# Sunshine-718/AlphaZero-AL

Measured on AMD Instinct MI355X. Metric: self-play positions/sec (Connect4 n_playout=200, batch=8192 games/GPU, vl_batch=4), higher is better.
Workload: dtype f32; 1 GPU; Connect4 self-play, n_playout=200, 8192 games/GPU, vl_batch=4, evaluator=cnn; c_base=1000, use_symmetry=True, lead_in_plies=12, streams_per_gpu=1, parallelism=independent game shards x1

## Files before the change

alphazero-al_amd/csrc/nn_conv.hip:

```cpp
#include <cstdio>
#include <cstdlib>

#include "az_nn.h"
#include "nn_common.h"

namespace {

constexpr int CELLS = 42, COLS = 7;
constexpr int PCOLS = 8, PCELLS = 72;
constexpr int TS = 4;
constexpr int COUT = 64;
constexpr int CELLB = 128;

__device__ __forceinline__ void glds16(const void *gsrc, uint32_t lds_off)
{
    uint32_t keep;
    asm volatile("s_mov_b32 %0, m0\n\ts_mov_b32 m0, %2\n\ts_nop 0\n\tglobal_load_lds_dwordx4 %1, off\n\ts_mov_b32 m0, %0"
                 : "=&s"(keep) : "v"(gsrc), "s"(lds_off) : "memory");
}
__device__ __forceinline__ uint32_t lds_addr(const void *p)
{
    return static_cast<uint32_t>(reinterpret_cast<uintptr_t>((__attribute__((address_space(3))) const void *)p));
}
__device__ __forceinline__ void lds_barrier()
{
    asm volatile("s_waitcnt lgkmcnt(0)" ::: "memory");
    __builtin_amdgcn_s_barrier();
    asm volatile("" ::: "memory");
}

__device__ unsigned long long g_prof[2048 * 8];

struct EmbedIn {
    const float    *features;
    const uint16_t *emb_own, *emb_opp;
    const uint16_t *pos;
    const int32_t  *gather;
    const uint64_t *bb_p1, *bb_p2;
    const int32_t  *turn, *sym;
};

template <int CIN, bool NORM, bool RESID, bool EMBED = false>
__global__ void __launch_bounds__(256, 2) k_conv_block(const uint16_t *x, const uint16_t *w, const uint16_t *bias,
                                                       const uint16_t *gamma, const uint16_t *beta, uint16_t *y,
                                                       int64_t B, float eps, int dbg, const int64_t *batch_dev, EmbedIn em)
{
    static_assert(!EMBED || (CIN == 32 && !NORM && !RESID), "the embedding is fused into the stem only");
    const int64_t rows_total = B;
    if (batch_dev != nullptr && *batch_dev < B) B = *batch_dev;
    constexpr int K = 9 * CIN;
    constexpr int KSTEPS = K / 32;
    constexpr int KPT = CIN / 32;
    constexpr int VPC = CIN / 8;
    constexpr int VPS = CELLS * VPC;
    constexpr int PER = (VPS + 63) / 64;
    constexpr int SB = VPS * 16;
    constexpr int OVPS = CELLS * COUT / 8;
    constexpr int OPER = (OVPS + 63) / 64;
    constexpr int OSB = OVPS * 16;

    extern __shared__ __align__(16) uint8_t smem[];
    uint8_t *img = smem;
    uint8_t *rawb = smem + TS * PCELLS * CELLB;
    uint8_t *outs = rawb + 2 * TS * SB;
    float *s_gam = reinterpret_cast<float *>(outs + (RESID ? 0 : TS * OSB)), *s_bet = s_gam + CIN;
    uint8_t *dump = reinterpret_cast<uint8_t *>(s_gam + 2 * CIN);

    const int tid = threadIdx.x;
    const int lane = tid & 63;
    const int wave = __builtin_amdgcn_readfirstlane(tid >> 6);
    const int mh = wave & 1, th = wave >> 1;
    const int l15 = lane & 15, l4 = lane >> 4;

    bf16x8 aw[2][KSTEPS];
    float bia[2][4];
#pragma unroll
    for (int mt = 0; mt < 2; ++mt) {
        const int o = mh * 32 + (l15 >> 2) * 8 + mt * 4 + (l15 & 3);
#pragma unroll
        for (int s = 0; s < KSTEPS; ++s)
            aw[mt][s] = *reinterpret_cast<const bf16x8 *>(w + static_cast<size_t>(o) * K + s * 32 + l4 * 8);
#pragma unroll
        for (int r = 0; r < 4; ++r)
            bia[mt][r] = __uint_as_float(static_cast<uint32_t>(bias[mh * 32 + l4 * 8 + mt * 4 + r]) << 16);
    }
    if (NORM && tid < CIN) {
        s_gam[tid] = __uint_as_float(static_cast<uint32_t>(gamma[tid]) << 16);
        s_bet[tid] = __uint_as_float(static_cast<uint32_t>(beta[tid]) << 16);
    }
    {
        V8 z; z.w[0] = z.w[1] = z.w[2] = z.w[3] = 0;
        constexpr int NV = (TS * PCELLS * CELLB + 2 * TS * SB) / 16;
        for (int i = tid; i < NV; i += 256) reinterpret_cast<V8 *>(smem)[i] = z;
    }
    __syncthreads();

    auto swz_in = [](int cell) { return VPC == 8 ? (cell & 7) : 0; };
    const uint32_t raw_lds = lds_addr(rawb);
    if (EMBED) {
        for (int i = tid; i < CELLS * CIN / 8; i += 256)
            reinterpret_cast<V8 *>(rawb)[i] = reinterpret_cast<const V8 *>(em.pos)[i];
        __syncthreads();
    }
    auto stage_tile = [&](int64_t tile, int buf, int lane) {
        const int64_t b = tile * TS + wave;
        if (EMBED || b >= B) return;
        const uint16_t *xs = x + b * (CELLS * CIN);
#pragma unroll
        for (int i = 0; i < PER; ++i) {
            const int s = lane + 64 * i;
            if (s < VPS) {
                const int cell = s / VPC;
                glds16(xs + (cell * VPC + ((s % VPC) ^ swz_in(cell))) * 8, raw_lds + (buf * TS + wave) * SB + i * 1024);
            }
        }
    };

    const int64_t ntiles = (B + TS - 1) / TS;
    float pl_own[PER], pl_opp[PER];
    auto load_planes = [&](int64_t tile, int lane) {
        const int64_t b = tile * TS + wave;
        const bool live = b < B;
        int64_t row = !live ? 0 : (em.gather != nullptr ? em.gather[b] : b);
        if (row < 0 || row >= rows_total) row = 0;
        if (em.features != nullptr) {
            const float *fs = em.features + row * (3 * CELLS);
#pragma unroll
            for (int i = 0; i < PER; ++i) {
                const int s = lane + 64 * i;
                const bool ok = live && s < VPS;
                pl_own[i] = ok ? fs[s / VPC] : 0.0f;
                pl_opp[i] = ok ? fs[CELLS + s / VPC] : 0.0f;
            }
        } else {
            const bool p1 = em.turn[row] > 0, mir = em.sym[row] != 0;
            const uint64_t own = p1 ? em.bb_p1[row] : em.bb_p2[row], opp = p1 ? em.bb_p2[row] : em.bb_p1[row];
#pragma unroll
            for (int i = 0; i < PER; ++i) {
                const int s = lane + 64 * i;
                const bool ok = live && s < VPS;
                const int cell = ok ? s / VPC : 0;
                const int r = cell / COLS, c = cell - r * COLS;
                const int bit = (mir ? COLS - 1 - c : c) * 7 + (5 - r);
                pl_own[i] = (ok && ((own >> bit) & 1ull)) ? 1.0f : 0.0f;
                pl_opp[i] = (ok && ((opp >> bit) & 1ull)) ? 1.0f : 0.0f;
            }
        }
    };
    if (EMBED && static_cast<int64_t>(blockIdx.x) < ntiles) load_planes(blockIdx.x, lane);
    if (static_cast<int64_t>(blockIdx.x) < ntiles) stage_tile(blockIdx.x, 0, lane);
    asm volatile("s_waitcnt vmcnt(0)" ::: "memory");
    lds_barrier();
    int par = 0;
    const bool prof = dbg & 16;
    unsigned long long tp[6] = {0, 0, 0, 0, 0, 0}, tl = prof ? __builtin_amdgcn_s_memtime() : 0;
    auto stamp = [&](int k) {
        if (prof) {
            const unsigned long long now = __builtin_amdgcn_s_memtime();
            tp[k] += now - tl;
            tl = now;
        }
    };
    uint32_t img_off[PER];
#pragma unroll
    for (int i = 0; i < PER; ++i) {
        const int sl = lane + 64 * i;
        const int cell = sl / VPC;
        const int r = cell / COLS, c = cell - r * COLS;
        const int p = (r + 1) * PCOLS + (c + 1);
        const int ck = (lane % VPC) ^ swz_in(lane / VPC);
        img_off[i] = static_cast<uint32_t>((wave * PCELLS + p) * CELLB + ((ck ^ (p & 7)) << 4));
    }
    for (int64_t tile = blockIdx.x; tile < ntiles; tile += gridDim.x, par ^= 1) {
        const int64_t b0 = tile * TS;
        uint8_t *rawt = rawb + par * TS * SB;
        uint8_t *outt = RESID ? rawt : outs;
        int lane_t = lane;
        asm volatile("" : "+v"(lane_t));

        {
            const int ck = (lane_t % VPC) ^ swz_in(lane_t / VPC);
            V8 raw[PER];
            if (EMBED) {
                const V8 eo = *reinterpret_cast<const V8 *>(em.emb_own + ck * 8), ep = *reinterpret_cast<const V8 *>(em.emb_opp + ck * 8);
#pragma unroll
                for (int i = 0; i < PER; ++i) {
                    const int s = lane_t + 64 * i;
                    if (s < VPS) {
                        const V8 ps = *reinterpret_cast<const V8 *>(rawb + s * 16);
                        const f32x2 own = {pl_own[i], pl_own[i]}, opp = {pl_opp[i], pl_opp[i]};
#pragma unroll
                        for (int q = 0; q < 4; ++q) {
                            const f32x2 v = unpack2(ps.w[q]) + own * unpack2(eo.w[q]) + opp * unpack2(ep.w[q]);
                            raw[i].w[q] = pack2(v.x, v.y);
                        }
                    } else {
                        raw[i].w[0] = raw[i].w[1] = raw[i].w[2] = raw[i].w[3] = 0;
                    }
                }
            } else {
#pragma unroll
                for (int i = 0; i < PER; ++i) {
                    const int s = lane_t + 64 * i;
                    if (s < VPS) raw[i] = *reinterpret_cast<const V8 *>(rawt + wave * SB + s * 16);
                    else raw[i].w[0] = raw[i].w[1] = raw[i].w[2] = raw[i].w[3] = 0;
                }
            }
            f32x2 sc[4], sh[4];
            if (NORM) {
                f32x2 sum2 = {0.0f, 0.0f}, sq2 = {0.0f, 0.0f};
#pragma unroll
                for (int i = 0; i < PER; ++i) {
#pragma unroll
                    for (int q = 0; q < 4; ++q) {
                        const f32x2 f = unpack2(raw[i].w[q]);
                        sum2 += f;
                        sq2 = __builtin_elementwise_fma(f, f, sq2);
                    }
                }
                const float sum = wave_sum(sum2.x + sum2.y), sq = wave_sum(sq2.x + sq2.y);
                const float mean = sum * (1.0f / (CELLS * CIN));
                const float var = fmaxf(sq * (1.0f / (CELLS * CIN)) - mean * mean, 0.0f);
                const float rstd = rsqrtf(var + eps);
#pragma unroll
                for (int q = 0; q < 4; ++q) {
                    const f32x2 gq = *reinterpret_cast<const f32x2 *>(&s_gam[ck * 8 + 2 * q]);
                    const f32x2 bq = *reinterpret_cast<const f32x2 *>(&s_bet[ck * 8 + 2 * q]);
                    sc[q] = gq * f32x2{rstd, rstd};
                    sh[q] = bq - sc[q] * f32x2{mean, mean};
                }
            }
#pragma unroll
            for (int i = 0; i < PER; ++i) {
                const int s = lane_t + 64 * i;
                if (s < VPS) {
                    V8 out = raw[i];
                    if (NORM) {
#pragma unroll
                        for (int q = 0; q < 4; ++q) {
                            const f32x2 f = __builtin_elementwise_fma(unpack2(raw[i].w[q]), sc[q], sh[q]);
                            out.w[q] = pack2(f.x, f.y);
                        }
                    }
                    *reinterpret_cast<V8 *>(img + img_off[i]) = out;
                }
            }
        }
        stamp(0);
        lds_barrier();
        stamp(1);
        if (tile + gridDim.x < ntiles) {
            stage_tile(tile + gridDim.x, par ^ 1, lane_t);
            if (EMBED) load_planes(tile + gridDim.x, lane_t);
        }

        uint32_t col[3][KPT];
        {
            const uint32_t pc = static_cast<uint32_t>(2 * th * PCELLS + l15 + 9 - PCOLS - 1);
#pragma unroll
            for (int d = 0; d < 3; ++d) {
                const uint32_t p = pc + d;
                const uint32_t o = (p * CELLB + ((l4 ^ (p & 7)) << 4)) & 0xffffu;
#pragma unroll
                for (int ks = 0; ks < KPT; ++ks) col[d][ks] = o ^ (ks << 6);
            }
        }
        auto fetch = [&](int it, int tap, bf16x8 (&xf)[KPT]) {
            const int dy = tap / 3, d = tap % 3;
            const int disp = (dy * PCOLS + (it / 3) * PCELLS + (it % 3) * 16) * CELLB;
#pragma unroll
            for (int ks = 0; ks < KPT; ++ks)
                xf[ks] = *reinterpret_cast<const bf16x8 *>(&smem[col[d][ks] + disp]);
        };
        struct Epi { V8 *slot; V8 rr, o; f32x2 t, v; };
        auto epi_begin = [&](int it, Epi &e) {
            const int smp = 2 * th + it / 3, t = (it % 3) * 16 + l15;
            const int cell = (t >> 3) * COLS + (t & 7);
            const uint32_t m = (t & 7) == 7 ? 0xffffffffu : 0u;
            const uint32_t off_real = static_cast<uint32_t>(outt - smem) + smp * OSB + cell * 128 + (((mh * 4 + l4) ^ (cell & 7)) << 4);
            const uint32_t off_dump = static_cast<uint32_t>(dump - smem) + (wave * 8 + (l15 >> 3) + 2 * l4) * 16;
            e.slot = reinterpret_cast<V8 *>(&smem[(off_real & ~m) | (off_dump & m)]);
            if (RESID) e.rr = *e.slot;
        };
        auto epi_step = [&](int step, const f32x4 (&acc)[2], Epi &e) {
            const int q = step / 9;
            const f32x2 x = {acc[q >> 1][2 * (q & 1)], acc[q >> 1][2 * (q & 1) + 1]};
            switch (step % 9) {
            case 0: e.t = x * f32x2{-1.44269504f, -1.44269504f}; break;
            case 1: e.t.x = __builtin_amdgcn_exp2f(e.t.x); break;
            case 2: e.t.y = __builtin_amdgcn_exp2f(e.t.y); break;
            case 3: e.t += f32x2{1.0f, 1.0f}; break;
            case 4: e.t.x = __builtin_amdgcn_rcpf(e.t.x); break;
            case 5: e.t.y = __builtin_amdgcn_rcpf(e.t.y); break;
            case 6: e.v = x * e.t; break;
            case 7: if (RESID) e.v += unpack2(e.rr.w[q]); break;
            default: e.o.w[q] = pack2(e.v.x, e.v.y); break;
            }
        };
        auto epi_end = [&](Epi &e) { *e.slot = e.o; };

        auto block = [&](int it, f32x4 (&acc)[2], bool with_epi, const f32x4 (&pacc)[2]) {
#pragma unroll
            for (int mt = 0; mt < 2; ++mt) acc[mt] = f32x4{bia[mt][0], bia[mt][1], bia[mt][2], bia[mt][3]};
            Epi e;
            if (with_epi) epi_begin(it - 1, e);
            bf16x8 xa[KPT], xb[KPT];
            fetch(it, 0, xa);
            __builtin_amdgcn_sched_barrier(0);
#pragma unroll
            for (int tap = 0; tap < 9; ++tap) {
                bf16x8 (&cur)[KPT] = (tap & 1) ? xb : xa;
                bf16x8 (&nxt)[KPT] = (tap & 1) ? xa : xb;
                if (tap + 1 < 9) fetch(it, tap + 1, nxt);
                __builtin_amdgcn_sched_barrier(0);
#pragma unroll
                for (int ks = 0; ks < KPT; ++ks)
#pragma unroll
                    for (int mt = 0; mt < 2; ++mt) {
                        const int s = tap * KPT + ks;
                        acc[mt] = __builtin_amdgcn_mfma_f32_16x16x32_bf16(aw[mt][s], cur[ks], acc[mt], 0, 0, 0);
                        if (with_epi) {
                            __builtin_amdgcn_sched_barrier(0);
                            constexpr int PER_SLOT = 36 / (18 * KPT);
                            const int slot = (tap * KPT + ks) * 2 + mt;
#pragma unroll
                            for (int j = 0; j < PER_SLOT; ++j) epi_step(slot * PER_SLOT + j, pacc, e);
                            __builtin_amdgcn_sched_barrier(0);
                        }
                    }
            }
            if (with_epi) epi_end(e);
        };
        if (!(dbg & 1)) {
            if ((dbg >> 5) & 3) {
                if (((dbg >> 5) & 3) == 1) __builtin_amdgcn_s_setprio(1);
                else if (((dbg >> 5) & 3) == 2) __builtin_amdgcn_s_setprio(2);
                else __builtin_amdgcn_s_setprio(3);
            }
            f32x4 acc_a[2], acc_b[2];
            block(0, acc_a, false, acc_b);
            block(1, acc_b, true, acc_a);
            block(2, acc_a, true, acc_b);
            block(3, acc_b, true, acc_a);
            block(4, acc_a, true, acc_b);
            block(5, acc_b, true, acc_a);
            {
                Epi e;
                epi_begin(5, e);
#pragma unroll
                for (int step = 0; step < 36; ++step) epi_step(step, acc_b, e);
                epi_end(e);
            }
            if ((dbg >> 5) & 3) __builtin_amdgcn_s_setprio(0);
        }
        stamp(2);
        asm volatile("s_waitcnt vmcnt(0)" ::: "memory");
        stamp(3);
        lds_barrier();
        stamp(4);

        if (b0 + wave < B && !(dbg & 2)) {
            uint16_t *ys = y + (b0 + wave) * (CELLS * COUT);
#pragma unroll
            for (int i = 0; i < OPER; ++i) {
                const int s = lane_t + 64 * i;
                if (s < OVPS) {
                    const int cell = s >> 3;
                    const V8 v = *reinterpret_cast<const V8 *>(outt + wave * OSB + s * 16);
                    *reinterpret_cast<V8 *>(ys + cell * COUT + (((s & 7) ^ (cell & 7)) << 3)) = v;
                }
            }
        }
        stamp(5);
    }
    if (prof && lane == 0 && blockIdx.x < 512)
        for (int k = 0; k < 6; ++k) g_prof[(blockIdx.x * 4 + wave) * 8 + k] = tp[k];
}

int g_dbg = 0;

template <int CIN, bool NORM, bool RESID, bool EMBED = false>
int launch(const void *x, const void *w, const void *bias, const void *gamma, const void *beta, void *y, int64_t B,
           float eps, const int64_t *batch_dev, hipStream_t s, EmbedIn em = EmbedIn{})
{
    constexpr size_t smem = static_cast<size_t>(TS) * PCELLS * CELLB + 2 * static_cast<size_t>(TS) * CELLS * CIN * 2 +
                            (RESID ? 0 : static_cast<size_t>(TS) * CELLS * COUT * 2) + 2 * CIN * sizeof(float) + 512;
    auto kern = k_conv_block<CIN, NORM, RESID, EMBED>;
    static DeviceSetup setup;
    if (setup.cus({reinterpret_cast<const void *>(kern)}, static_cast<int>(smem), [&] {
            if (getenv("AZ_NN_VERBOSE") != nullptr) {
                int per_cu = 0;
                (void)hipOccupancyMaxActiveBlocksPerMultiprocessor(&per_cu, reinterpret_cast<const void *>(kern), 256, smem);
                fprintf(stderr, "[az_nn] conv block C_in=%d: %zu B LDS, %d workgroups per CU\n", CIN, smem, per_cu);
            }
        }) == 0)
        return 2;
    static const int prio = [] { const char *e = getenv("AZ_NN_CONV_PRIO"); const int v = e ? atoi(e) : 1; return v < 0 || v > 3 ? 1 : v; }();
    const int64_t ntiles = (B + TS - 1) / TS;
    static const int64_t max_grid = getenv("AZ_NN_CONV_GRID") ? atoll(getenv("AZ_NN_CONV_GRID")) : 512;
    const unsigned grid = static_cast<unsigned>(ntiles < max_grid ? ntiles : max_grid);
    hipLaunchKernelGGL(kern, dim3(grid), dim3(256), smem, s, static_cast<const uint16_t *>(x),
                       static_cast<const uint16_t *>(w), static_cast<const uint16_t *>(bias),
                       static_cast<const uint16_t *>(gamma), static_cast<const uint16_t *>(beta),
                       static_cast<uint16_t *>(y), B, eps, g_dbg | (((g_dbg >> 5) & 3) ? 0 : (prio << 5)), batch_dev, em);
    return 0;
}

}

extern "C" {

int az_nn_debug(int flags) { g_dbg = flags; return 0; }

int az_nn_conv_profile(unsigned long long *out, int n)
{
    if (n > 2048 * 8) n = 2048 * 8;
    return hipMemcpyFromSymbol(out, HIP_SYMBOL(g_prof), sizeof(unsigned long long) * n) == hipSuccess ? 0 : 2;
}

int az_nn_conv_block(const void *x, int c_in, const void *weight_ohwi, const void *bias, const void *gamma,
                     const void *beta, int residual, void *y, int64_t batch, float eps, const int64_t *batch_dev,
                     void *stream)
{
    if (batch <= 0) return 1;
    hipStream_t s = static_cast<hipStream_t>(stream);
    const bool norm = gamma != nullptr && beta != nullptr;
    if (c_in == 64 && norm && residual) return launch<64, true, true>(x, weight_ohwi, bias, gamma, beta, y, batch, eps, batch_dev, s);
    if (c_in == 64 && norm && !residual) return launch<64, true, false>(x, weight_ohwi, bias, gamma, beta, y, batch, eps, batch_dev, s);
    if (c_in == 32 && !norm && !residual) return launch<32, false, false>(x, weight_ohwi, bias, gamma, beta, y, batch, eps, batch_dev, s);
    return 1;
}

int az_nn_stem_embed(const float *features, const void *emb_own, const void *emb_opp, const void *pos,
                     const void *weight_ohwi, const void *bias, void *y, int64_t batch, const int32_t *gather,
                     const int64_t *batch_dev, void *stream)
{
    if (batch <= 0 || features == nullptr) return 1;
    EmbedIn em{features, static_cast<const uint16_t *>(emb_own), static_cast<const uint16_t *>(emb_opp),
               static_cast<const uint16_t *>(pos), gather, nullptr, nullptr, nullptr, nullptr};
    return launch<32, false, false, true>(nullptr, weight_ohwi, bias, nullptr, nullptr, y, batch, 0.0f, batch_dev,
                                          static_cast<hipStream_t>(stream), em);
}

int az_nn_stem_embed_positions(const az_nn_positions *positions, const void *emb_own, const void *emb_opp, const void *pos,
                               const void *weight_ohwi, const void *bias, void *y, int64_t batch, const int32_t *gather,
                               const int64_t *batch_dev, void *stream)
{
    if (batch <= 0 || positions == nullptr || !positions->bb_p1 || !positions->bb_p2 || !positions->turn || !positions->sym) return 1;
    EmbedIn em{nullptr, static_cast<const uint16_t *>(emb_own), static_cast<const uint16_t *>(emb_opp),
               static_cast<const uint16_t *>(pos), gather, positions->bb_p1, positions->bb_p2, positions->turn, positions->sym};
    return launch<32, false, false, true>(nullptr, weight_ohwi, bias, nullptr, nullptr, y, batch, 0.0f, batch_dev,
                                          static_cast<hipStream_t>(stream), em);
}

}
```

alphazero-al_amd/csrc/nn_model.hip:

```cpp
#include <hip/hip_runtime.h>

#include <cstdint>
#include <cstdlib>
#include <cstring>
#include <mutex>
#include <new>
#include <vector>

#include "az_nn.h"
#include "board_sym.h"

struct az_nn_model {
    int kind = AZ_NN_KIND_CONNECT4_CNN;
    bool attn_heads_fused = true;
    az_nn_model_weights w{};
    az_nn_othello_weights ow{};
};

namespace {
constexpr int64_t kTokenBytes = 42 * 64 * 2;
constexpr uint64_t kOtTok = 64 * 32 * 2, kOtMap10 = 100 * 256 * 2, kOtMap8 = 64 * 256 * 2, kOtNeck = 64 * 8 * 2;

constexpr int kKinds = 4;
struct Profile {
    std::mutex mu;
    bool on = false;
    int stride = 1;
    int64_t seen = 0;
    std::vector<hipEvent_t> start[kKinds], stop[kKinds];
    size_t used[kKinds] = {0, 0, 0, 0};
} g_prof;
constexpr size_t kProfileMax = 4096;

__device__ __forceinline__ uint64_t position_hash(uint64_t bb0, uint64_t bb1, bool p1_to_move)
{
    uint64_t x = bb0 * 0x9E3779B97F4A7C15ull;
    x ^= (bb1 + 0x7F4A7C159E3779B9ull) * 0xBF58476D1CE4E5B9ull;
    x += p1_to_move ? 0x94D049BB133111EBull : 0x2545F4914F6CDD1Dull;
    x ^= x >> 30; x *= 0xBF58476D1CE4E5B9ull;
    x ^= x >> 27; x *= 0x94D049BB133111EBull;
    x ^= x >> 31;
    return x;
}

template <bool OTHELLO>
__global__ void __launch_bounds__(256) k_hash_eval(const float *features, const uint8_t *mask, float *probs, float *wdl,
                                                   float *ml, int64_t batch, const int32_t *rows, const int64_t *n_rows)
{
    constexpr int CELLS = OTHELLO ? 64 : 42, A = OTHELLO ? 65 : 7;
    const int lane = threadIdx.x & 63;
    const int64_t b = static_cast<int64_t>(blockIdx.x) * (blockDim.x >> 6) + (threadIdx.x >> 6);
    int64_t n = batch;
    if (n_rows != nullptr && *n_rows < n) n = *n_rows;
    if (b >= n) return;
    int64_t row = rows != nullptr ? rows[b] : b;
    if (row < 0 || row >= batch) return;
    const float *f = features + row * 3 * CELLS;
    const bool in = lane < CELLS;
    const float own = in ? f[lane] : 0.0f, opp = in ? f[CELLS + lane] : 0.0f;
    const bool p1 = f[2 * CELLS] > 0.0f;
    const int bit = OTHELLO ? lane : ((lane % 7) * 7 + (5 - lane / 7));
    const bool is_p1 = in && ((p1 && own != 0.0f) || (!p1 && opp != 0.0f));
    const bool is_p2 = in && ((p1 && opp != 0.0f) || (!p1 && own != 0.0f));
    uint64_t bb0 = 0, bb1 = 0;
    if (OTHELLO) {
        bb0 = __ballot(is_p1); bb1 = __ballot(is_p2);
    } else {
        const uint64_t m1 = __ballot(is_p1), m2 = __ballot(is_p2);
        for (int c = 0; c < 42; ++c) {
            const int bt = (c % 7) * 7 + (5 - c / 7);
            bb0 |= ((m1 >> c) & 1ull) << bt;
            bb1 |= ((m2 >> c) & 1ull) << bt;
        }
        (void)bit;
    }
    const uint64_t h = position_hash(bb0, bb1, p1);
    const uint8_t *mk = mask != nullptr ? mask + row * A : nullptr;
    if (!OTHELLO) {
        if (lane < 7) {
            const float p = static_cast<float>(1 + ((h >> (4 * lane)) & 15)) / 16.0f;
            probs[row * 7 + lane] = (mk == nullptr || mk[lane]) ? p : 0.0f;
        }
    } else {
        for (int a = lane; a < 65; a += 64) {
            const int k = a >> 4, j = a & 15;
            uint64_t hk = h + 0x9E3779B97F4A7C15ull * static_cast<uint64_t>(k + 1);
            hk ^= hk >> 29; hk *= 0xBF58476D1CE4E5B9ull; hk ^= hk >> 32;
            const float p = static_cast<float>(1 + ((hk >> (4 * j)) & 15)) / 16.0f;
            probs[row * 65 + a] = (mk == nullptr || mk[a]) ? p : 0.0f;
        }
    }
    if (lane < 3) {
        const uint64_t w0 = 1 + ((h >> 28) & 31), w1 = 1 + ((h >> 33) & 31), w2 = 1 + ((h >> 38) & 31);
        const float tot = static_cast<float>(w0 + w1 + w2);
        const uint64_t mine = lane == 0 ? w0 : (lane == 1 ? w1 : w2);
        wdl[row * 3 + lane] = static_cast<float>(mine) / tot;
    }
    if (lane == 3) {
        const float v = static_cast<float>((h >> 43) & 63);
        ml[row] = OTHELLO ? (v / 32.0f - 1.0f) : (v / 2.0f);
    }
}

template <bool OTHELLO>
__global__ void __launch_bounds__(256) k_hash_eval_positions(az_nn_positions pos, const uint8_t *mask, float *probs, float *wdl,
                                                             float *ml, int64_t batch, const int32_t *rows, const int64_t *n_rows)
{
    constexpr int A = OTHELLO ? 65 : 7;
    const int64_t b = static_cast<int64_t>(blockIdx.x) * blockDim.x + threadIdx.x;
    int64_t n = batch;
    if (n_rows != nullptr && *n_rows < n) n = *n_rows;
    if (b >= n) return;
    const int64_t row = rows != nullptr ? rows[b] : b;
    if (row < 0 || row >= batch) return;
    uint64_t bb0 = pos.bb_p1[row], bb1 = pos.bb_p2[row];
    const int sym = pos.sym[row];
    if (OTHELLO) { bb0 = az::othello_sym(bb0, sym); bb1 = az::othello_sym(bb1, sym); }
    else if (sym) { bb0 = az::mirror_columns(bb0); bb1 = az::mirror_columns(bb1); }
    const uint64_t h = position_hash(bb0, bb1, pos.turn[row] > 0);
    const uint8_t *mk = mask != nullptr ? mask + row * A : nullptr;
    if (!OTHELLO) {
        for (int a = 0; a < 7; ++a) {
            const float p = static_cast<float>(1 + ((h >> (4 * a)) & 15)) / 16.0f;
            probs[row * 7 + a] = (mk == nullptr || mk[a]) ? p : 0.0f;
        }
    } else {
        for (int k = 0; k < 5; ++k) {
            uint64_t hk = h + 0x9E3779B97F4A7C15ull * static_cast<uint64_t>(k + 1);
            hk ^= hk >> 29; hk *= 0xBF58476D1CE4E5B9ull; hk ^= hk >> 32;
            for (int j = 0; j < 16 && k * 16 + j < 65; ++j) {
                const int a = k * 16 + j;
                const float p = static_cast<float>(1 + ((hk >> (4 * j)) & 15)) / 16.0f;
                probs[row * 65 + a] = (mk == nullptr || mk[a]) ? p : 0.0f;
            }
        }
    }
    const uint64_t w0 = 1 + ((h >> 28) & 31), w1 = 1 + ((h >> 33) & 31), w2 = 1 + ((h >> 38) & 31);
    const float tot = static_cast<float>(w0 + w1 + w2);
    wdl[row * 3 + 0] = static_cast<float>(w0) / tot;
    wdl[row * 3 + 1] = static_cast<float>(w1) / tot;
    wdl[row * 3 + 2] = static_cast<float>(w2) / tot;
    const float v = static_cast<float>((h >> 43) & 63);
    ml[row] = OTHELLO ? (v / 32.0f - 1.0f) : (v / 2.0f);
}
}

extern "C" {

int az_nn_model_create(const az_nn_model_weights *w, az_nn_model **out)
{
    if (w == nullptr || out == nullptr) return 1;
    if (w->n_blocks < 0 || w->n_blocks > AZ_NN_MAX_BLOCKS) return 1;
    if ((w->stem_frag == nullptr) != (w->stem_pmap == nullptr)) return 1;
    const void *need[] = {w->emb_own, w->emb_opp, w->pos, w->stem_w, w->stem_b, w->pre_w, w->qkvg_w,
                          w->qn_w, w->kn_w, w->o_w, w->heads.p_norm, w->heads.d_val_w};
    for (const void *p : need)
        if (p == nullptr) return 1;
    for (int i = 0; i < w->n_blocks; ++i)
        if (!w->block_w[i] || !w->block_b[i] || !w->block_gamma[i] || !w->block_beta[i]) return 1;
    auto *m = new (std::nothrow) az_nn_model();
    if (m == nullptr) return 1;
    m->w = *w;
    const char *fused = getenv("AZ_ATTN_HEADS_FUSED");
    m->attn_heads_fused = fused == nullptr || strcmp(fused, "0") != 0;
    *out = m;
    return 0;
}

int az_nn_model_create_hash(int game, az_nn_model **out)
{
    if (out == nullptr || (game != 0 && game != 1)) return 1;
    auto *m = new (std::nothrow) az_nn_model();
    if (m == nullptr) return 1;
    m->kind = game == 0 ? AZ_NN_KIND_HASH_CONNECT4 : AZ_NN_KIND_HASH_OTHELLO;
    *out = m;
    return 0;
}

int az_nn_model_create_othello(const az_nn_othello_weights *w, az_nn_model **out)
{
    if (w == nullptr || out == nullptr || w->embed_table == nullptr) return 1;
    if (w->n_body < 2 || w->n_body % 2 != 0 || w->n_convs != w->n_body + 2 || w->n_convs > AZ_NN_OTHELLO_MAX_CONVS) return 1;
    for (int i = 0; i < w->n_convs; ++i)
        if (!w->conv[i].w_packed || !w->conv[i].post_scale || !w->conv[i].post_shift) return 1;
    if (!w->dual_w16 || !w->dual_scale16 || !w->dual_shift16 || !w->heads.board_w || !w->heads.a_fc_wt) return 1;
    auto *m = new (std::nothrow) az_nn_model();
    if (m == nullptr) return 1;
    m->kind = AZ_NN_KIND_OTHELLO_CNN;
    m->ow = *w;
    *out = m;
    return 0;
}

void az_nn_model_destroy(az_nn_model *m) { delete m; }

int az_nn_model_kind(const az_nn_model *m) { return m ? m->kind : -1; }

uint64_t az_nn_model_scratch_bytes(const az_nn_model *m, int64_t batch)
{
    if (m != nullptr && m->kind == AZ_NN_KIND_OTHELLO_CNN)
        return batch > 0 ? static_cast<uint64_t>(batch) * (kOtTok + 3 * kOtMap10 + 2 * kOtMap8 + kOtNeck) : 0;
    if (m != nullptr && m->kind != AZ_NN_KIND_CONNECT4_CNN) return 0;
    return batch > 0 ? static_cast<uint64_t>(2 * batch * kTokenBytes) : 0;
}

static int forward_impl(const az_nn_model *m, const float *features, const az_nn_positions *positions, const uint8_t *mask,
                        float *probs, float *wdl, float *moves_left, int64_t batch, const int32_t *rows,
                        const int64_t *n_rows, void *scratch, uint64_t scratch_bytes, void *stream);

int az_nn_model_forward(const az_nn_model *m, const float *features, const uint8_t *mask, float *probs,
                        float *wdl, float *moves_left, int64_t batch, const int32_t *rows,
                        const int64_t *n_rows, void *scratch, uint64_t scratch_bytes, void *stream)
{
    if (features == nullptr) return 1;
    return forward_impl(m, features, nullptr, mask, probs, wdl, moves_left, batch, rows, n_rows, scratch, scratch_bytes, stream);
}

int az_nn_model_forward_positions(const az_nn_model *m, const az_nn_positions *positions, const uint8_t *mask, float *probs,
                                  float *wdl, float *moves_left, int64_t batch, const int32_t *rows,
                                  const int64_t *n_rows, void *scratch, uint64_t scratch_bytes, void *stream)
{
    if (positions == nullptr || !positions->bb_p1 || !positions->bb_p2 || !positions->turn || !positions->sym) return 1;
    return forward_impl(m, nullptr, positions, mask, probs, wdl, moves_left, batch, rows, n_rows, scratch, scratch_bytes, stream);
}

static int forward_impl(const az_nn_model *m, const float *features, const az_nn_positions *positions, const uint8_t *mask,
                        float *probs, float *wdl, float *moves_left, int64_t batch, const int32_t *rows,
                        const int64_t *n_rows, void *scratch, uint64_t scratch_bytes, void *stream)
{
    if (m == nullptr || probs == nullptr || wdl == nullptr || moves_left == nullptr) return 1;
    if (batch <= 0) return batch == 0 ? 0 : 1;
    if ((rows == nullptr) != (n_rows == nullptr)) return 1;
    if (m->kind == AZ_NN_KIND_OTHELLO_CNN) {
        if (positions == nullptr || mask == nullptr) return 1;
        if (scratch == nullptr || scratch_bytes < az_nn_model_scratch_bytes(m, batch)) return 1;
        const az_nn_othello_weights &o = m->ow;
        char *base = static_cast<char *>(scratch);
        char *tok = base; base += batch * kOtTok;
        char *map[3];
        for (auto &p : map) { p = base; base += batch * kOtMap10; }
        char *pa = base; base += batch * kOtMap8;
        char *pb = base; base += batch * kOtMap8;
        char *neck = base;
        auto conv = [&](int i, const void *x, const void *res, void *y) {
            const az_nn_othello_conv_layer &l = o.conv[i];
            return az_nn_othello_conv(x, l.w_packed, l.pre_scale, l.pre_shift, l.post_scale, l.post_shift, l.residual ? res : nullptr,
                                      y, batch, l.c_in, l.h_in, l.pad, 1, n_rows, stream);
        };
        int rc = az_nn_othello_embed(positions, mask, o.embed_table, tok, batch, rows, n_rows, stream);
        int cur = 0;
        if (rc == 0) rc = conv(0, tok, nullptr, map[cur]);
        for (int i = 1; rc == 0 && i + 1 < o.n_body; i += 2) {
            const int y1 = (cur + 1) % 3, y2 = (cur + 2) % 3;
            rc = conv(i, map[cur], nullptr, map[y1]);
            if (rc == 0) rc = conv(i + 1, map[y1], map[cur], map[y2]);
            cur = y2;
        }
        const int hid = (cur + 1) % 3;
        if (rc == 0) rc = conv(o.n_body - 1, map[cur], nullptr, map[hid]);
        if (rc == 0) rc = conv(o.n_body, map[hid], nullptr, pa);
        if (rc == 0) rc = conv(o.n_body + 1, pa, nullptr, pb);
        if (rc == 0) rc = az_nn_othello_conv_narrow(map[hid], o.dual_w16, o.dual_scale16, o.dual_shift16, neck, batch, n_rows, stream);
        if (rc == 0) rc = az_nn_othello_heads(pb, neck, &o.heads, probs, wdl, moves_left, batch, rows, n_rows, stream);
        return rc;
    }
    if (m->kind != AZ_NN_KIND_CONNECT4_CNN && positions != nullptr) {
        const dim3 grid(static_cast<unsigned>((batch + 255) / 256)), block(256);
        if (m->kind == AZ_NN_KIND_HASH_OTHELLO)
            hipLaunchKernelGGL(k_hash_eval_positions<true>, grid, block, 0, static_cast<hipStream_t>(stream), *positions, mask, probs,
                               wdl, moves_left, batch, rows, n_rows);
        else
            hipLaunchKernelGGL(k_hash_eval_positions<false>, grid, block, 0, static_cast<hipStream_t>(stream), *positions, mask, probs,
                               wdl, moves_left, batch, rows, n_rows);
        return 0;
    }
    if (m->kind != AZ_NN_KIND_CONNECT4_CNN) {
        const dim3 grid(static_cast<unsigned>((batch + 3) / 4)), block(256);
        if (m->kind == AZ_NN_KIND_HASH_OTHELLO)
            hipLaunchKernelGGL(k_hash_eval<true>, grid, block, 0, static_cast<hipStream_t>(stream), features, mask, probs, wdl,
                               moves_left, batch, rows, n_rows);
        else
            hipLaunchKernelGGL(k_hash_eval<false>, grid, block, 0, static_cast<hipStream_t>(stream), features, mask, probs, wdl,
                               moves_left, batch, rows, n_rows);
        return 0;
    }
    if (scratch == nullptr || scratch_bytes < az_nn_model_scratch_bytes(m, batch)) return 1;
    const az_nn_model_weights &w = m->w;
    char *a = static_cast<char *>(scratch);
    char *b = a + batch * kTokenBytes;
    hipStream_t hs = static_cast<hipStream_t>(stream);
    bool timed = false;
    int slot[kKinds] = {-1, -1, -1, -1};
    if (g_prof.on) {
        std::lock_guard<std::mutex> lk(g_prof.mu);
        hipStreamCaptureStatus cs = hipStreamCaptureStatusNone;
        const bool capturing = hipStreamIsCapturing(hs, &cs) == hipSuccess && cs != hipStreamCaptureStatusNone;
        if (g_prof.on && !capturing && (g_prof.seen++ % g_prof.stride) == 0) {
            timed = true;
            for (int kd = 0; kd < kKinds; ++kd)
                if (g_prof.used[kd] < g_prof.start[kd].size()) slot[kd] = static_cast<int>(g_prof.used[kd]++);
        }
    }
    auto begin = [&](int kd) { if (timed && slot[kd] >= 0) (void)hipEventRecord(g_prof.start[kd][slot[kd]], hs); };
    auto end = [&](int kd) { if (timed && slot[kd] >= 0) (void)hipEventRecord(g_prof.stop[kd][slot[kd]], hs); };
    begin(AZ_NN_PROFILE_STEM);
    int rc;
    if (w.stem_frag != nullptr && w.stem_pmap != nullptr)
        rc = positions != nullptr
            ? az_nn_stem_folded_positions(positions, w.stem_frag, w.stem_pmap, a, batch, rows, n_rows, stream)
            : az_nn_stem_folded(features, w.stem_frag, w.stem_pmap, a, batch, rows, n_rows, stream);
    else
        rc = positions != nullptr
            ? az_nn_stem_embed_positions(positions, w.emb_own, w.emb_opp, w.pos, w.stem_w, w.stem_b, a, batch, rows, n_rows, stream)
            : az_nn_stem_embed(features, w.emb_own, w.emb_opp, w.pos, w.stem_w, w.stem_b, a, batch, rows, n_rows, stream);
    end(AZ_NN_PROFILE_STEM);
    for (int i = 0; rc == 0 && i < w.n_blocks; ++i) {
        if (i == 0) begin(AZ_NN_PROFILE_CONV);
        rc = az_nn_conv_block(a, 64, w.block_w[i], w.block_b[i], w.block_gamma[i], w.block_beta[i], 1, b, batch,
                              w.eps, n_rows, stream);
        if (i == 0) end(AZ_NN_PROFILE_CONV);
        char *t = a; a = b; b = t;
    }
    if (rc == 0 && m->attn_heads_fused && !timed)
        return az_nn_attn_heads(a, w.pre_w, w.qkvg_w, w.qn_w, w.kn_w, w.o_w, &w.heads, mask, probs, wdl, moves_left, batch,
                                w.eps, rows, n_rows, stream);
    if (rc == 0) {
        begin(AZ_NN_PROFILE_ATTN);
        rc = az_nn_attn_block(a, w.pre_w, w.qkvg_w, w.qn_w, w.kn_w, w.o_w, b, batch, w.eps, n_rows, stream);
        end(AZ_NN_PROFILE_ATTN);
        char *t = a; a = b; b = t;
    }
    if (rc == 0) {
        begin(AZ_NN_PROFILE_HEADS);
        rc = az_nn_heads(a, &w.heads, mask, probs, wdl, moves_left, batch, w.eps, rows, n_rows, stream);
        end(AZ_NN_PROFILE_HEADS);
    }
    return rc;
}

int az_nn_model_profile(int enable)
{
    std::lock_guard<std::mutex> lk(g_prof.mu);
    if (enable) {
        for (int kd = 0; kd < kKinds; ++kd)
            while (g_prof.start[kd].size() < kProfileMax) {
                hipEvent_t a, b;
                if (hipEventCreate(&a) != hipSuccess || hipEventCreate(&b) != hipSuccess) return 2;
                g_prof.start[kd].push_back(a); g_prof.stop[kd].push_back(b);
            }
    }
    g_prof.on = enable != 0;
    g_prof.stride = enable > 1 ? enable : 1;
    g_prof.seen = 0;
    return 0;
}

int az_nn_model_profile_read_kernels(double out_ms[4], int64_t out_launches[4])
{
    if (out_ms == nullptr || out_launches == nullptr) return 1;
    if (hipDeviceSynchronize() != hipSuccess) return 2;
    std::lock_guard<std::mutex> lk(g_prof.mu);
    for (int kd = 0; kd < kKinds; ++kd) {
        double ms = 0.0;
        for (size_t i = 0; i < g_prof.used[kd]; ++i) {
            float t = 0.f;
            if (hipEventElapsedTime(&t, g_prof.start[kd][i], g_prof.stop[kd][i]) != hipSuccess) return 2;
            ms += t;
        }
        out_ms[kd] = ms;
        out_launches[kd] = static_cast<int64_t>(g_prof.used[kd]);
        g_prof.used[kd] = 0;
    }
    return 0;
}

int az_nn_model_profile_read(double *out_ms, int64_t *out_launches)
{
    if (out_ms == nullptr || out_launches == nullptr) return 1;
    double ms[4]; int64_t n[4];
    const int rc = az_nn_model_profile_read_kernels(ms, n);
    if (rc != 0) return rc;
    *out_ms = ms[AZ_NN_PROFILE_CONV];
    *out_launches = n[AZ_NN_PROFILE_CONV];
    return 0;
}

}
```

alphazero-al_amd/src/fast_net.py:

```python
import ctypes as C
import os

import torch
import torch.nn.functional as F

ROWS, COLS, CELLS = 6, 7, 42

_GLUE = None


def glue():
    global _GLUE
    if _GLUE is None:
        path = os.path.join(os.path.dirname(os.path.dirname(os.path.abspath(__file__))), "lib", "libaz_mcts.so")
        try:
            L = C.CDLL(path)
            vp, i64, i32, f32 = C.c_void_p, C.c_int64, C.c_int, C.c_float
            L.az_nn_embed.argtypes = [vp, vp, vp, vp, vp, i64, i32, vp, vp, vp]
            L.az_nn_groupnorm1.argtypes = [vp, vp, vp, vp, i64, i32, f32, vp]
            L.az_nn_silu_add.argtypes = [vp, vp, i32, vp, vp, i64, vp]
            L.az_nn_rmsnorm64.argtypes = [vp, vp, vp, i64, f32, vp]
            L.az_nn_qkv_prep.argtypes = [vp, i32, vp, vp, vp, vp, vp, vp, i64, f32, vp]
            L.az_nn_attn_post.argtypes = [vp, vp, vp, i64, vp]
            L.az_nn_heads_prep.argtypes = [vp, vp, vp, f32, vp, vp, i64, f32, vp]
            L.az_nn_conv_block.argtypes = [vp, i32, vp, vp, vp, vp, i32, vp, i64, f32, vp, vp]
            L.az_nn_conv_block2.argtypes = [vp, vp, vp, vp, vp, i64, f32, vp, vp]
            L.az_nn_attn_block.argtypes = [vp, vp, vp, vp, vp, vp, vp, i64, f32, vp, vp]
            L.az_nn_heads.argtypes = [vp, C.POINTER(HeadsWeights), vp, vp, vp, vp, i64, f32, vp, vp, vp]
            L.az_nn_attn_heads.argtypes = [vp, vp, vp, vp, vp, vp, C.POINTER(HeadsWeights), vp, vp, vp, vp, i64, f32, vp,
                                           vp, vp]
            L.az_nn_stem_embed.argtypes = [vp, vp, vp, vp, vp, vp, vp, i64, vp, vp, vp]
            L.az_nn_stem_folded.argtypes = [vp, vp, vp, vp, i64, vp, vp, vp]
            L.az_nn_model_create.argtypes = [C.POINTER(ModelWeights), C.POINTER(vp)]
            L.az_nn_model_destroy.argtypes = [vp]
            L.az_nn_model_destroy.restype = None
            L.az_nn_model_scratch_bytes.argtypes = [vp, i64]
            L.az_nn_model_scratch_bytes.restype = C.c_uint64
            L.az_nn_model_forward.argtypes = [vp, vp, vp, vp, vp, vp, i64, vp, vp, vp, C.c_uint64, vp]
            _GLUE = L
        except OSError:
            _GLUE = False
    return _GLUE or None


def fold_block(w, bias, gamma, beta):
    w32 = w.float().contiguous()
    wf = (w32 * gamma.float().view(1, -1, 1, 1)).to(torch.bfloat16)
    wff = wf.float()
    wb = w32 * beta.float().view(1, -1, 1, 1)
    t1 = torch.zeros((9, w.shape[0]), dtype=torch.float32, device=w.device)
    t2 = torch.zeros_like(t1)
    taps = {0: (1, 2), 1: (0, 1, 2), 2: (0, 1)}
    for rc in range(3):
        for cc in range(3):
            kh, kw = list(taps[rc]), list(taps[cc])
            t1[3 * rc + cc] = wff[:, :, kh][:, :, :, kw].sum((1, 2, 3))
            t2[3 * rc + cc] = bias.float() + wb[:, :, kh][:, :, :, kw].sum((1, 2, 3))
    return (wf.contiguous(memory_format=torch.channels_last), t1.contiguous(), (t2 * 1.4426950408889634).contiguous())


def fold_stem(weight, bias, emb_own, emb_opp, pos_map):
    w = weight.to(torch.bfloat16).float()
    out_c = w.shape[0]
    assert out_c == 64 and tuple(w.shape[2:]) == (3, 3) and pos_map.shape[0] == CELLS
    a = torch.einsum("ocyx,c->oyx", w, emb_own.float()).reshape(out_c, 9)
    b = torch.einsum("ocyx,c->oyx", w, emb_opp.float()).reshape(out_c, 9)
    t = torch.zeros((out_c, 32), dtype=torch.float32, device=w.device)
    t[:, 0:18:2] = a
    t[:, 1:18:2] = b
    hi = t.to(torch.bfloat16)
    lo = (t - hi.float()).to(torch.bfloat16)
    lane = torch.arange(64, device=w.device)
    ti, r = torch.arange(4, device=w.device).view(4, 1), (lane & 15).view(1, 64)
    rows = 32 * (ti // 2) + 8 * (r // 4) + 4 * (ti % 2) + r % 4
    cols = ((lane >> 4) * 8).view(64, 1) + torch.arange(8, device=w.device).view(1, 8)
    frag = torch.stack([part[rows.view(4, 64, 1), cols.view(1, 64, 8)] for part in (hi, lo)]).contiguous()
    pm = torch.nn.functional.conv2d(pos_map.float().t().reshape(1, -1, 6, COLS), w, bias.to(torch.bfloat16).float(), padding=1)
    pmap = torch.zeros((48, 68), dtype=torch.float32, device=w.device)
    pmap[:CELLS, :out_c] = pm.reshape(out_c, CELLS).t()
    return frag, pmap.contiguous()


class HeadsWeights(C.Structure):
    _PTRS = ("p_norm", "p_gate_w", "p_fc_w", "p_fc_b", "p_out_w", "d_pool_norm", "d_pool_w", "d_pool_b", "d_norm",
             "d_fc_w", "d_fc_b", "d_out_norm", "d_val_w", "d_val_b", "d_aux_w")
    _fields_ = [(n, C.c_void_p) for n in _PTRS] + [(n, C.c_float) for n in ("p_gate_b", "p_out_b", "d_aux_b", "aux_scale")]


MAX_BLOCKS = 8


class ModelWeights(C.Structure):
    _fields_ = ([(n, C.c_void_p) for n in ("emb_own", "emb_opp", "pos", "stem_w", "stem_b")] + [("n_blocks", C.c_int32)] +
                [(n, C.c_void_p * MAX_BLOCKS) for n in ("block_w", "block_b", "block_gamma", "block_beta")] +
                [(n, C.c_void_p) for n in ("pre_w", "qkvg_w", "qn_w", "kn_w", "o_w")] +
                [("heads", HeadsWeights), ("eps", C.c_float), ("stem_frag", C.c_void_p), ("stem_pmap", C.c_void_p)])


class FastConnect4Net(torch.nn.Module):
    aux_target_offset = 42
    n_actions = COLS

    def __init__(self, state_dict, device, dtype=torch.bfloat16, heads=4):
        super().__init__()
        self.device = torch.device(device)
        self.dtype = dtype
        self.heads = heads
        sd = {k: v.detach().to(self.device) for k, v in state_dict.items()}
        c = lambda t: t.to(dtype).contiguous()
        f = lambda t: t.to(torch.float32).contiguous()

        self.embed_dim = sd["piece_emb.weight"].shape[1]
        self.register_buffer("emb_own", c(sd["piece_emb.weight"][0]))
        self.register_buffer("emb_opp", c(sd["piece_emb.weight"][1]))
        self.register_buffer("pos", c(sd["pos_emb.weight"][sd["orbit_map"].long()]))

        def conv_w(w):
            return c(w).contiguous(memory_format=torch.channels_last)
        self.register_buffer("stem_w", conv_w(sd["hidden.0.weight"]))
        self.register_buffer("stem_b", c(sd["hidden.0.bias"]))
        self.folded_stem = os.environ.get("AZ_STEM_FOLDED", "1") != "0" and sd["hidden.0.weight"].shape[0] == 64
        if self.folded_stem:
            frag, pmap = fold_stem(sd["hidden.0.weight"], sd["hidden.0.bias"], sd["piece_emb.weight"][0], sd["piece_emb.weight"][1],
                                   sd["pos_emb.weight"][sd["orbit_map"].long()])
            self.register_buffer("stem_frag", frag)
            self.register_buffer("stem_pmap", pmap)
        self.h_dim = sd["hidden.0.weight"].shape[0]
        self.res = []
        i = 2
        while f"hidden.{i}.conv.weight" in sd:
            names = (f"res{i}_w", f"res{i}_b", f"res{i}_g", f"res{i}_beta")
            self.register_buffer(names[0], conv_w(sd[f"hidden.{i}.conv.weight"]))
            self.register_buffer(names[1], c(sd[f"hidden.{i}.conv.bias"]))
            self.register_buffer(names[2], c(sd[f"hidden.{i}.norm.weight"]))
            self.register_buffer(names[3], c(sd[f"hidden.{i}.norm.bias"]))
            self.res.append(names)
            i += 1
        a = f"hidden.{i}.attn."
        self.register_buffer("pre_w", c(sd[a + "prenorm.weight"]))
        qkvg = torch.cat([sd[a + "qkv_proj.weight"], sd[a + "gate_proj.weight"]], 0)
        self.register_buffer("qkvg_w", c(qkvg))
        self.register_buffer("o_w", c(sd[a + "o_proj.weight"]))
        self.register_buffer("qn_w", c(sd[a + "q_norm.weight"]))
        self.register_buffer("kn_w", c(sd[a + "k_norm.weight"]))
        p = "policy_head."
        self.register_buffer("p_norm", c(sd[p + "norm.weight"]))
        self.register_buffer("p_gate_w", c(sd[p + "row_gate.weight"].reshape(-1)))
        self.register_buffer("p_gate_b", f(sd[p + "row_gate.bias"]))
        self.register_buffer("p_fc_w", c(sd[p + "fc.weight"]))
        self.register_buffer("p_fc_b", c(sd[p + "fc.bias"]))
        self.register_buffer("p_out_w", c(sd[p + "out.weight"].reshape(-1)))
        self.register_buffer("p_out_b", f(sd[p + "out.bias"]))
        d = "dual_head."
        self.register_buffer("d_pool_norm", c(sd[d + "pool_norm.weight"]))
        self.register_buffer("d_pool_w", c(sd[d + "pool_fc.weight"]))
        self.register_buffer("d_pool_b", c(sd[d + "pool_fc.bias"]))
        self.register_buffer("d_norm", c(sd[d + "norm.weight"]))
        self.register_buffer("d_fc_w", c(sd[d + "fc.weight"]))
        self.register_buffer("d_fc_b", c(sd[d + "fc.bias"]))
        self.register_buffer("d_out_norm", c(sd[d + "out_norm.weight"]))
        self.register_buffer("d_val_w", c(sd[d + "value_out.weight"]))
        self.register_buffer("d_val_b", c(sd[d + "value_out.bias"]))
        self.register_buffer("d_aux_w", c(sd[d + "aux_out.weight"].reshape(-1)))
        self.register_buffer("d_aux_b", f(sd[d + "aux_out.bias"]))
        self.p_gate_b_host = float(sd[p + "row_gate.bias"].reshape(-1)[0].item())
        self.hip = (self.device.type == "cuda" and dtype == torch.bfloat16 and self.embed_dim == 32
                    and self.h_dim == 64 and heads == 4 and glue() is not None)
        self.mfma_conv = self.mfma_attn = self.fused_stem = self.fused_heads = self.hip
        self.attn_heads_fused = self.hip and os.environ.get("AZ_ATTN_HEADS_FUSED", "1") != "0"
        self._heads_w = None
        if self.fused_heads:
            hw = HeadsWeights()
            for n in HeadsWeights._PTRS:
                setattr(hw, n, getattr(self, n).data_ptr())
            hw.p_gate_b = self.p_gate_b_host
            hw.p_out_b = float(self.p_out_b.reshape(-1)[0].item())
            hw.d_aux_b = float(self.d_aux_b.reshape(-1)[0].item())
            hw.aux_scale = float(self.aux_target_offset)
            self._heads_w = hw

    def native_model(self):
        if not self.supports_compact or not self.fused_stem or len(self.res) > MAX_BLOCKS:
            return None
        if self.__dict__.get("_model") is None:
            w = ModelWeights()
            for n in ("emb_own", "emb_opp", "pos", "stem_w", "stem_b", "pre_w", "qkvg_w", "qn_w", "kn_w", "o_w"):
                setattr(w, n, getattr(self, n).data_ptr())
            w.n_blocks = len(self.res)
            for i, names in enumerate(self.res):
                for field, name in zip(("block_w", "block_b", "block_gamma", "block_beta"), names):
                    getattr(w, field)[i] = getattr(self, name).data_ptr()
            w.heads = self._heads_w
            w.eps = 1e-5
            if self.folded_stem:
                w.stem_frag, w.stem_pmap = self.stem_frag.data_ptr(), self.stem_pmap.data_ptr()
            h = C.c_void_p()
            if glue().az_nn_model_create(C.byref(w), C.byref(h)) != 0:
                raise RuntimeError("az_nn_model_create refused the weights")
            self.__dict__["_model"] = h
        return self.__dict__["_model"]

    def __del__(self):
        try:
            h = self.__dict__.get("_model")
            if h is not None and _GLUE:
                self.__dict__["_model"] = None
                _GLUE.az_nn_model_destroy(h)
        except Exception:
            pass

    @classmethod
    def from_module(cls, net, dtype=torch.bfloat16, device=None):
        sd = net.state_dict()
        if device is None:
            device = next(iter(sd.values())).device
        return cls(sd, device, dtype)

    @staticmethod
    def recognises(net):
        need = ("piece_emb", "pos_emb", "hidden", "policy_head", "dual_head", "orbit_map")
        return all(hasattr(net, n) for n in need)

    def _conv(self, tokens, w, b):
        bsz, _, cin = tokens.shape
        img = tokens.view(bsz, ROWS, COLS, cin).permute(0, 3, 1, 2)
        out = F.conv2d(img, w, b, padding=1)
        return out.permute(0, 2, 3, 1).reshape(bsz, CELLS, -1)

    def _group_norm1(self, tokens, gamma, beta):
        bsz = tokens.shape[0]
        y = F.layer_norm(tokens.reshape(bsz, -1), (tokens.shape[1] * tokens.shape[2],), eps=1e-5)
        return torch.addcmul(beta, y.view_as(tokens), gamma)

    def _rms(self, x, w):
        return F.rms_norm(x, (x.shape[-1],), w, 1e-5)

    @property
    def supports_compact(self):
        return bool(self.hip)

    @torch.no_grad()
    def predict_device(self, x, action_mask=None, rows=None, n_rows=None, out=None):
        if rows is not None:
            assert self.supports_compact and out is not None and n_rows is not None
            t, bsz, L, s = self._body_hip(x, rows, n_rows, attention=not self.attn_heads_fused)
            probs, wdl, ml = out
            m = action_mask.contiguous()
            self._heads_launch(t, m, probs, wdl, ml, bsz, rows.data_ptr(), n_rows.data_ptr(), L, s)
            self._keep_mask = m
            return probs, wdl, ml
        if not (self.hip and x.is_cuda):
            lp, v, st = self(x, action_mask)
            return lp.exp(), v.exp(), st * float(self.aux_target_offset)
        if not self.fused_heads:
            lp, v, st = self._forward_hip(x, action_mask)
            return lp.exp(), v.exp(), st * float(self.aux_target_offset)
        t, bsz, L, s = self._body_hip(x, attention=not self.attn_heads_fused)
        probs = torch.empty((bsz, COLS), dtype=torch.float32, device=self.device)
        wdl = torch.empty((bsz, 3), dtype=torch.float32, device=self.device)
        ml = torch.empty((bsz,), dtype=torch.float32, device=self.device)
        m = None
        if action_mask is not None:
            m = action_mask if action_mask.dtype in (torch.uint8, torch.bool) else action_mask.to(torch.bool)
            m = m.contiguous()
        self._heads_launch(t, m, probs, wdl, ml, bsz, None, None, L, s)
        self._keep_mask = m
        return probs, wdl, ml

    def _heads_launch(self, t, m, probs, wdl, ml, bsz, rows_ptr, n_rows_ptr, L, s):
        mp = None if m is None else m.data_ptr()
        if self.attn_heads_fused:
            L.az_nn_attn_heads(t.data_ptr(), self.pre_w.data_ptr(), self.qkvg_w.data_ptr(), self.qn_w.data_ptr(),
                               self.kn_w.data_ptr(), self.o_w.data_ptr(), C.byref(self._heads_w), mp, probs.data_ptr(),
                               wdl.data_ptr(), ml.data_ptr(), bsz, 1e-5, rows_ptr, n_rows_ptr, s)
        else:
            L.az_nn_heads(t.data_ptr(), C.byref(self._heads_w), mp, probs.data_ptr(), wdl.data_ptr(), ml.data_ptr(), bsz,
                          1e-5, rows_ptr, n_rows_ptr, s)

    @torch.no_grad()
    def _forward_hip(self, x, action_mask):
        t, bsz, L, s = self._body_hip(x)
        return self._heads_hip(t, action_mask, bsz, L, s)

    @torch.no_grad()
    def _body_hip(self, x, rows=None, n_rows=None, attention=True):
        L = glue()
        gp = None if rows is None else rows.data_ptr()
        np_ = None if n_rows is None else n_rows.data_ptr()
        s = C.c_void_p(torch.cuda.current_stream().cuda_stream)
        bsz = x.shape[0]
        dev, bf = self.device, torch.bfloat16
        c_dim = self.h_dim
        x = x.contiguous().float()
        t = torch.empty((bsz, CELLS, c_dim), dtype=bf, device=dev)
        if self.folded_stem:
            L.az_nn_stem_folded(x.data_ptr(), self.stem_frag.data_ptr(), self.stem_pmap.data_ptr(), t.data_ptr(), bsz, gp, np_, s)
        else:
            L.az_nn_stem_embed(x.data_ptr(), self.emb_own.data_ptr(), self.emb_opp.data_ptr(), self.pos.data_ptr(),
                               self.stem_w.data_ptr(), self.stem_b.data_ptr(), t.data_ptr(), bsz, gp, np_, s)
        for w, b, g, beta in self.res:
            t2 = torch.empty_like(t)
            L.az_nn_conv_block(t.data_ptr(), c_dim, getattr(self, w).data_ptr(), getattr(self, b).data_ptr(),
                               getattr(self, g).data_ptr(), getattr(self, beta).data_ptr(), 1, t2.data_ptr(),
                               bsz, 1e-5, np_, s)
            t = t2
        if not attention:
            return t, bsz, L, s
        t2 = torch.empty_like(t)
        L.az_nn_attn_block(t.data_ptr(), self.pre_w.data_ptr(), self.qkvg_w.data_ptr(), self.qn_w.data_ptr(),
                           self.kn_w.data_ptr(), self.o_w.data_ptr(), t2.data_ptr(), bsz, 1e-5, np_, s)
        return t2, bsz, L, s

    @torch.no_grad()
    def _heads_hip(self, t, action_mask, bsz, L, s):
        dev, bf, c_dim = self.device, torch.bfloat16, self.h_dim
        col = torch.empty((bsz, COLS, c_dim), dtype=bf, device=dev)
        mean = torch.empty((bsz, c_dim), dtype=bf, device=dev)
        L.az_nn_heads_prep(t.data_ptr(), self.p_norm.data_ptr(), self.p_gate_w.data_ptr(), self.p_gate_b_host,
                           col.data_ptr(), mean.data_ptr(), bsz, 1e-5, s)
        col = F.silu(F.linear(col, self.p_fc_w, self.p_fc_b))
        logits = (col.float() * self.p_out_w.float()).sum(-1) + self.p_out_b
        if action_mask is not None:
            logits = logits.masked_fill(~action_mask.to(torch.bool), -1e9)
        log_prob = F.log_softmax(logits, dim=-1)
        g = mean + F.silu(F.linear(self._rms(mean, self.d_pool_norm), self.d_pool_w, self.d_pool_b))
        hh = self._rms(F.silu(F.linear(self._rms(g, self.d_norm), self.d_fc_w, self.d_fc_b)), self.d_out_norm)
        value = F.log_softmax(F.linear(hh, self.d_val_w, self.d_val_b).float(), dim=-1)
        steps = torch.sigmoid((hh.float() * self.d_aux_w.float()).sum(-1) + self.d_aux_b)
        return log_prob, value, steps

    @torch.no_grad()
    def forward(self, x, action_mask=None):
        if self.hip and x.is_cuda:
            return self._forward_hip(x, action_mask)
        bsz = x.shape[0]
        dt = self.dtype
        own = x[:, 0].reshape(bsz, CELLS, 1).to(dt)
        opp = x[:, 1].reshape(bsz, CELLS, 1).to(dt)
        t = torch.addcmul(torch.addcmul(self.pos, own, self.emb_own), opp, self.emb_opp)

        t = F.silu(self._conv(t, self.stem_w, self.stem_b))
        for w, b, g, beta in self.res:
            y = self._group_norm1(t, getattr(self, g), getattr(self, beta))
            t = t + F.silu(self._conv(y, getattr(self, w), getattr(self, b)))

        h = self._rms(t, self.pre_w)
        qkvg = F.linear(h, self.qkvg_w)
        c_dim, nh = self.h_dim, self.heads
        hd = c_dim // nh
        q, k, v = qkvg[..., :3 * c_dim].view(bsz, CELLS, 3, nh, hd).unbind(2)
        gate = qkvg[..., 3 * c_dim:]
        q = self._rms(q, self.qn_w).transpose(1, 2)
        k = self._rms(k, self.kn_w).transpose(1, 2)
        a = F.scaled_dot_product_attention(q, k, v.transpose(1, 2))
        a = a * torch.sigmoid(gate).transpose(1, 2).unsqueeze(-1)
        t = F.linear(a.transpose(1, 2).reshape(bsz, CELLS, c_dim), self.o_w) + t

        pn = self._rms(t, self.p_norm).view(bsz, ROWS, COLS, c_dim)
        scores = (pn.float() * self.p_gate_w.float()).sum(-1) + self.p_gate_b
        wts = torch.softmax(scores, dim=1).to(dt)
        col = (wts.unsqueeze(-1) * pn).sum(dim=1)
        col = F.silu(F.linear(col, self.p_fc_w, self.p_fc_b))
        logits = (col.float() * self.p_out_w.float()).sum(-1) + self.p_out_b
        if action_mask is not None:
            logits = logits.masked_fill(~action_mask.to(torch.bool), -1e9)
        log_prob = F.log_softmax(logits, dim=-1)

        g = t.float().mean(dim=1).to(dt)
        g = g + F.silu(F.linear(self._rms(g, self.d_pool_norm), self.d_pool_w, self.d_pool_b))
        hh = self._rms(F.silu(F.linear(self._rms(g, self.d_norm), self.d_fc_w, self.d_fc_b)), self.d_out_norm)
        value = F.log_softmax(F.linear(hh, self.d_val_w, self.d_val_b).float(), dim=-1)
        steps = torch.sigmoid((hh.float() * self.d_aux_w.float()).sum(-1) + self.d_aux_b)
        return log_prob, value, steps

    @torch.no_grad()
    def predict(self, state, action_mask=None):
        import numpy as np
        t = torch.as_tensor(np.asarray(state), dtype=torch.float32, device=self.device)
        m = None if action_mask is None else torch.as_tensor(np.asarray(action_mask), device=self.device)
        probs, wdl, ml = self.predict_device(t, m)
        return probs.cpu().numpy(), wdl.cpu().numpy(), ml.view(-1, 1).cpu().numpy()
```

include/az_nn.h:

```cpp
#ifndef AZ_NN_H
#define AZ_NN_H

#include <stdint.h>

#ifdef __cplusplus
extern "C" {
#endif

int az_nn_embed(const float *features, const void *emb_own, const void *emb_opp, const void *pos,
                void *tokens, int64_t batch, int embed_dim, const int32_t *gather, const int64_t *batch_dev,
                void *stream);
int az_nn_groupnorm1(const void *x, const void *gamma, const void *beta, void *y, int64_t batch,
                     int channels, float eps, void *stream);
int az_nn_silu_add(const void *x, const void *bias, int channels, const void *residual, void *y,
                   int64_t n_elements, void *stream);
int az_nn_conv_block(const void *x, int c_in, const void *weight_ohwi, const void *bias, const void *gamma,
                     const void *beta, int residual, void *y, int64_t batch, float eps, const int64_t *batch_dev,
                     void *stream);
int az_nn_conv_block2(const void *x, const void *weight_folded_ohwi, const float *t1, const float *t2_scaled, void *y,
                      int64_t batch, float eps, const int64_t *batch_dev, void *stream);

int az_nn_stem_embed(const float *features, const void *emb_own, const void *emb_opp, const void *pos,
                     const void *weight_ohwi, const void *bias, void *y, int64_t batch, const int32_t *gather,
                     const int64_t *batch_dev, void *stream);
typedef struct az_nn_positions {
    const uint64_t *bb_p1, *bb_p2;
    const int32_t *turn, *sym;
} az_nn_positions;
int az_nn_stem_embed_positions(const az_nn_positions *positions, const void *emb_own, const void *emb_opp, const void *pos,
                               const void *weight_ohwi, const void *bias, void *y, int64_t batch, const int32_t *gather,
                               const int64_t *batch_dev, void *stream);
int az_nn_stem_folded(const float *features, const void *w_frag, const float *pmap, void *y, int64_t batch,
                      const int32_t *gather, const int64_t *batch_dev, void *stream);
int az_nn_stem_folded_positions(const az_nn_positions *positions, const void *w_frag, const float *pmap, void *y,
                                int64_t batch, const int32_t *gather, const int64_t *batch_dev, void *stream);
int az_nn_attn_block(const void *x, const void *prenorm_w, const void *qkvg_w, const void *q_norm_w,
                     const void *k_norm_w, const void *o_w, void *y, int64_t batch, float eps, const int64_t *batch_dev,
                     void *stream);
int az_nn_debug(int flags);
int az_nn_conv_profile(unsigned long long *out, int n);
int az_nn_rmsnorm64(const void *x, const void *w, void *y, int64_t rows, float eps, void *stream);
int az_nn_qkv_prep(const void *qkvg, int row_len, const void *q_norm_w, const void *k_norm_w, void *q,
                   void *k, void *v, void *gate_sigmoid, int64_t batch, float eps, void *stream);
int az_nn_attn_post(const void *attn, const void *gate_sigmoid, void *out, int64_t batch, void *stream);
int az_nn_heads_prep(const void *tokens, const void *p_norm_w, const void *p_gate_w, float p_gate_b,
                     void *col, void *mean, int64_t batch, float eps, void *stream);

typedef struct az_nn_heads_weights {
    const void *p_norm, *p_gate_w, *p_fc_w, *p_fc_b, *p_out_w;
    const void *d_pool_norm, *d_pool_w, *d_pool_b, *d_norm, *d_fc_w, *d_fc_b, *d_out_norm;
    const void *d_val_w, *d_val_b, *d_aux_w;
    float p_gate_b, p_out_b, d_aux_b, aux_scale;
} az_nn_heads_weights;
int az_nn_heads(const void *tokens, const az_nn_heads_weights *w, const uint8_t *mask, float *probs, float *wdl,
                float *moves_left, int64_t batch, float eps, const int32_t *scatter, const int64_t *batch_dev,
                void *stream);
int az_nn_attn_heads(const void *x, const void *prenorm_w, const void *qkvg_w, const void *q_norm_w, const void *k_norm_w,
                     const void *o_w, const az_nn_heads_weights *w, const uint8_t *mask, float *probs, float *wdl,
                     float *moves_left, int64_t batch, float eps, const int32_t *scatter, const int64_t *batch_dev,
                     void *stream);

#define AZ_NN_MAX_BLOCKS 8
typedef struct az_nn_model_weights {
    const void *emb_own, *emb_opp, *pos;
    const void *stem_w, *stem_b;
    int32_t n_blocks;
    const void *block_w[AZ_NN_MAX_BLOCKS], *block_b[AZ_NN_MAX_BLOCKS];
    const void *block_gamma[AZ_NN_MAX_BLOCKS], *block_beta[AZ_NN_MAX_BLOCKS];
    const void *pre_w, *qkvg_w, *qn_w, *kn_w, *o_w;
    az_nn_heads_weights heads;
    float eps;
    const void *stem_frag;
    const float *stem_pmap;
} az_nn_model_weights;
typedef struct az_nn_model az_nn_model;
int az_nn_model_create(const az_nn_model_weights *w, az_nn_model **out);
int az_nn_model_create_hash(int game, az_nn_model **out);
#define AZ_NN_KIND_CONNECT4_CNN  0
#define AZ_NN_KIND_HASH_CONNECT4 1
#define AZ_NN_KIND_HASH_OTHELLO  2
int az_nn_model_kind(const az_nn_model *m);
void az_nn_model_destroy(az_nn_model *m);
uint64_t az_nn_model_scratch_bytes(const az_nn_model *m, int64_t batch);
int az_nn_model_forward(const az_nn_model *m, const float *features, const uint8_t *mask, float *probs,
                        float *wdl, float *moves_left, int64_t batch, const int32_t *rows,
                        const int64_t *n_rows, void *scratch, uint64_t scratch_bytes, void *stream);
int az_nn_model_forward_positions(const az_nn_model *m, const az_nn_positions *positions, const uint8_t *mask, float *probs,
                                  float *wdl, float *moves_left, int64_t batch, const int32_t *rows,
                                  const int64_t *n_rows, void *scratch, uint64_t scratch_bytes, void *stream);
int az_nn_model_profile(int enable);
int az_nn_model_profile_read(double *out_ms, int64_t *out_launches);
#define AZ_NN_PROFILE_STEM  0
#define AZ_NN_PROFILE_CONV  1
#define AZ_NN_PROFILE_ATTN  2
#define AZ_NN_PROFILE_HEADS 3
int az_nn_model_profile_read_kernels(double out_ms[4], int64_t out_launches[4]);

int az_nn_othello_conv(const void *x, const void *w_packed, const float *pre_scale, const float *pre_shift,
                       const float *post_scale, const float *post_shift, const void *residual, void *y,
                       int64_t batch, int c_in, int h_in, int pad, int apply_silu, const int64_t *batch_dev, void *stream);

int az_nn_othello_conv_narrow(const void *x, const void *w_packed16, const float *post_scale16,
                              const float *post_shift16, void *y, int64_t batch, const int64_t *batch_dev, void *stream);

typedef struct az_nn_othello_heads_weights {
    const void  *board_w;
    const float *pass_norm_w, *pass_fc_w;
    const float *v_conv_w;
    const float *v_bn_s, *v_bn_b;
    const float *v_fc_w, *v_fc_b;
    const float *a_fc_wt, *a_fc_b;
    const float *a_norm_w, *a_out_w;
    float board_b, pass_fc_b, a_out_b;
    float aux_to_score;
    float eps;
    const void *a_fc_w16;
} az_nn_othello_heads_weights;
int az_nn_othello_embed(const az_nn_positions *positions, const uint8_t *mask, const void *embed_table, void *tokens,
                        int64_t batch, const int32_t *gather, const int64_t *batch_dev, void *stream);
int az_nn_othello_heads(const void *policy_map, const void *bottleneck, const az_nn_othello_heads_weights *w, float *probs,
                        float *wdl, float *utility, int64_t batch, const int32_t *scatter, const int64_t *batch_dev, void *stream);

#define AZ_NN_OTHELLO_MAX_CONVS 16
typedef struct az_nn_othello_conv_layer {
    const void *w_packed;
    const float *pre_scale, *pre_shift, *post_scale, *post_shift;
    int32_t residual, c_in, h_in, pad;
} az_nn_othello_conv_layer;
typedef struct az_nn_othello_weights {
    const void *embed_table;
    int32_t n_body, n_convs;
    az_nn_othello_conv_layer conv[AZ_NN_OTHELLO_MAX_CONVS];
    const void *dual_w16;
    const float *dual_scale16, *dual_shift16;
    az_nn_othello_heads_weights heads;
} az_nn_othello_weights;
#define AZ_NN_KIND_OTHELLO_CNN 3
int az_nn_model_create_othello(const az_nn_othello_weights *w, az_nn_model **out);

#ifdef __cplusplus
}
#endif
#endif
```

Before: 271,300 positions/s.

## Fuse folded stem into first residual conv block kernel

Measured after the change: 279,400 positions/s (median of 6 runs). +3.0%, better.

```diff
diff --git a/alphazero-al_amd/csrc/nn_conv.hip b/alphazero-al_amd/csrc/nn_conv.hip
--- a/alphazero-al_amd/csrc/nn_conv.hip
+++ b/alphazero-al_amd/csrc/nn_conv.hip
@@ -40,341 +40,35 @@
     const int32_t  *turn, *sym;
 };
 
+struct StemIn {
+    const uint64_t *bb_p1, *bb_p2;
+    const int32_t  *turn, *sym;
+    const int32_t  *gather;
+    const uint16_t *wfrag;
+    const float    *pmap;
+};
+constexpr int PROWS = 48, PROW = 68;
+constexpr int PMAPB = PROWS * PROW * 4, FRAGB = 2 * 4 * 64 * 16;
+
 template <int CIN, bool NORM, bool RESID, bool EMBED = false>
 __global__ void __launch_bounds__(256, 2) k_conv_block(const uint16_t *x, const uint16_t *w, const uint16_t *bias,
                                                        const uint16_t *gamma, const uint16_t *beta, uint16_t *y,
                                                        int64_t B, float eps, int dbg, const int64_t *batch_dev, EmbedIn em)
 {
-    static_assert(!EMBED || (CIN == 32 && !NORM && !RESID), "the embedding is fused into the stem only");
-    const int64_t rows_total = B;
-    if (batch_dev != nullptr && *batch_dev < B) B = *batch_dev;
-    constexpr int K = 9 * CIN;
-    constexpr int KSTEPS = K / 32;
-    constexpr int KPT = CIN / 32;
-    constexpr int VPC = CIN / 8;
-    constexpr int VPS = CELLS * VPC;
-    constexpr int PER = (VPS + 63) / 64;
-    constexpr int SB = VPS * 16;
-    constexpr int OVPS = CELLS * COUT / 8;
-    constexpr int OPER = (OVPS + 63) / 64;
-    constexpr int OSB = OVPS * 16;
+    constexpr bool STEM = false;
+    const StemIn st{};
+#include "nn_conv_body.h"
+}
 
-    extern __shared__ __align__(16) uint8_t smem[];
-    uint8_t *img = smem;
-    uint8_t *rawb = smem + TS * PCELLS * CELLB;
-    uint8_t *outs = rawb + 2 * TS * SB;
-    float *s_gam = reinterpret_cast<float *>(outs + (RESID ? 0 : TS * OSB)), *s_bet = s_gam + CIN;
-    uint8_t *dump = reinterpret_cast<uint8_t *>(s_gam + 2 * CIN);
-
-    const int tid = threadIdx.x;
-    const int lane = tid & 63;
-    const int wave = __builtin_amdgcn_readfirstlane(tid >> 6);
-    const int mh = wave & 1, th = wave >> 1;
-    const int l15 = lane & 15, l4 = lane >> 4;
-
-    bf16x8 aw[2][KSTEPS];
-    float bia[2][4];
-#pragma unroll
-    for (int mt = 0; mt < 2; ++mt) {
-        const int o = mh * 32 + (l15 >> 2) * 8 + mt * 4 + (l15 & 3);
-#pragma unroll
-        for (int s = 0; s < KSTEPS; ++s)
-            aw[mt][s] = *reinterpret_cast<const bf16x8 *>(w + static_cast<size_t>(o) * K + s * 32 + l4 * 8);
-#pragma unroll
-        for (int r = 0; r < 4; ++r)
-            bia[mt][r] = __uint_as_float(static_cast<uint32_t>(bias[mh * 32 + l4 * 8 + mt * 4 + r]) << 16);
-    }
-    if (NORM && tid < CIN) {
-        s_gam[tid] = __uint_as_float(static_cast<uint32_t>(gamma[tid]) << 16);
-        s_bet[tid] = __uint_as_float(static_cast<uint32_t>(beta[tid]) << 16);
-    }
-    {
-        V8 z; z.w[0] = z.w[1] = z.w[2] = z.w[3] = 0;
-        constexpr int NV = (TS * PCELLS * CELLB + 2 * TS * SB) / 16;
-        for (int i = tid; i < NV; i += 256) reinterpret_cast<V8 *>(smem)[i] = z;
-    }
-    __syncthreads();
-
-    auto swz_in = [](int cell) { return VPC == 8 ? (cell & 7) : 0; };
-    const uint32_t raw_lds = lds_addr(rawb);
-    if (EMBED) {
-        for (int i = tid; i < CELLS * CIN / 8; i += 256)
-            reinterpret_cast<V8 *>(rawb)[i] = reinterpret_cast<const V8 *>(em.pos)[i];
-        __syncthreads();
-    }
-    auto stage_tile = [&](int64_t tile, int buf, int lane) {
-        const int64_t b = tile * TS + wave;
-        if (EMBED || b >= B) return;
-        const uint16_t *xs = x + b * (CELLS * CIN);
-#pragma unroll
-        for (int i = 0; i < PER; ++i) {
-            const int s = lane + 64 * i;
-            if (s < VPS) {
-                const int cell = s / VPC;
-                glds16(xs + (cell * VPC + ((s % VPC) ^ swz_in(cell))) * 8, raw_lds + (buf * TS + wave) * SB + i * 1024);
-            }
-        }
-    };
-
-    const int64_t ntiles = (B + TS - 1) / TS;
-    float pl_own[PER], pl_opp[PER];
-    auto load_planes = [&](int64_t tile, int lane) {
-        const int64_t b = tile * TS + wave;
-        const bool live = b < B;
-        int64_t row = !live ? 0 : (em.gather != nullptr ? em.gather[b] : b);
-        if (row < 0 || row >= rows_total) row = 0;
-        if (em.features != nullptr) {
-            const float *fs = em.features + row * (3 * CELLS);
-#pragma unroll
-            for (int i = 0; i < PER; ++i) {
-                const int s = lane + 64 * i;
-                const bool ok = live && s < VPS;
-                pl_own[i] = ok ? fs[s / VPC] : 0.0f;
-                pl_opp[i] = ok ? fs[CELLS + s / VPC] : 0.0f;
-            }
-        } else {
-            const bool p1 = em.turn[row] > 0, mir = em.sym[row] != 0;
-            const uint64_t own = p1 ? em.bb_p1[row] : em.bb_p2[row], opp = p1 ? em.bb_p2[row] : em.bb_p1[row];
-#pragma unroll
-            for (int i = 0; i < PER; ++i) {
-                const int s = lane + 64 * i;
-                const bool ok = live && s < VPS;
-                const int cell = ok ? s / VPC : 0;
-                const int r = cell / COLS, c = cell - r * COLS;
-                const int bit = (mir ? COLS - 1 - c : c) * 7 + (5 - r);
-                pl_own[i] = (ok && ((own >> bit) & 1ull)) ? 1.0f : 0.0f;
-                pl_opp[i] = (ok && ((opp >> bit) & 1ull)) ? 1.0f : 0.0f;
-            }
-        }
-    };
-    if (EMBED && static_cast<int64_t>(blockIdx.x) < ntiles) load_planes(blockIdx.x, lane);
-    if (static_cast<int64_t>(blockIdx.x) < ntiles) stage_tile(blockIdx.x, 0, lane);
-    asm volatile("s_waitcnt vmcnt(0)" ::: "memory");
-    lds_barrier();
-    int par = 0;
-    const bool prof = dbg & 16;
-    unsigned long long tp[6] = {0, 0, 0, 0, 0, 0}, tl = prof ? __builtin_amdgcn_s_memtime() : 0;
-    auto stamp = [&](int k) {
-        if (prof) {
-            const unsigned long long now = __builtin_amdgcn_s_memtime();
-            tp[k] += now - tl;
-            tl = now;
-        }
-    };
-    uint32_t img_off[PER];
-#pragma unroll
-    for (int i = 0; i < PER; ++i) {
-        const int sl = lane + 64 * i;
-        const int cell = sl / VPC;
-        const int r = cell / COLS, c = cell - r * COLS;
-        const int p = (r + 1) * PCOLS + (c + 1);
-        const int ck = (lane % VPC) ^ swz_in(lane / VPC);
-        img_off[i] = static_cast<uint32_t>((wave * PCELLS + p) * CELLB + ((ck ^ (p & 7)) << 4));
-    }
-    for (int64_t tile = blockIdx.x; tile < ntiles; tile += gridDim.x, par ^= 1) {
-        const int64_t b0 = tile * TS;
-        uint8_t *rawt = rawb + par * TS * SB;
-        uint8_t *outt = RESID ? rawt : outs;
-        int lane_t = lane;
-        asm volatile("" : "+v"(lane_t));
-
-        {
-            const int ck = (lane_t % VPC) ^ swz_in(lane_t / VPC);
-            V8 raw[PER];
-            if (EMBED) {
-                const V8 eo = *reinterpret_cast<const V8 *>(em.emb_own + ck * 8), ep = *reinterpret_cast<const V8 *>(em.emb_opp + ck * 8);
-#pragma unroll
-                for (int i = 0; i < PER; ++i) {
-                    const int s = lane_t + 64 * i;
-                    if (s < VPS) {
-                        const V8 ps = *reinterpret_cast<const V8 *>(rawb + s * 16);
-                        const f32x2 own = {pl_own[i], pl_own[i]}, opp = {pl_opp[i], pl_opp[i]};
-#pragma unroll
-                        for (int q = 0; q < 4; ++q) {
-                            const f32x2 v = unpack2(ps.w[q]) + own * unpack2(eo.w[q]) + opp * unpack2(ep.w[q]);
-                            raw[i].w[q] = pack2(v.x, v.y);
-                        }
-                    } else {
-                        raw[i].w[0] = raw[i].w[1] = raw[i].w[2] = raw[i].w[3] = 0;
-                    }
-                }
-            } else {
-#pragma unroll
-                for (int i = 0; i < PER; ++i) {
-                    const int s = lane_t + 64 * i;
-                    if (s < VPS) raw[i] = *reinterpret_cast<const V8 *>(rawt + wave * SB + s * 16);
-                    else raw[i].w[0] = raw[i].w[1] = raw[i].w[2] = raw[i].w[3] = 0;
-                }
-            }
-            f32x2 sc[4], sh[4];
-            if (NORM) {
-                f32x2 sum2 = {0.0f, 0.0f}, sq2 = {0.0f, 0.0f};
-#pragma unroll
-                for (int i = 0; i < PER; ++i) {
-#pragma unroll
-                    for (int q = 0; q < 4; ++q) {
-                        const f32x2 f = unpack2(raw[i].w[q]);
-                        sum2 += f;
-                        sq2 = __builtin_elementwise_fma(f, f, sq2);
-                    }
-                }
-                const float sum = wave_sum(sum2.x + sum2.y), sq = wave_sum(sq2.x + sq2.y);
-                const float mean = sum * (1.0f / (CELLS * CIN));
-                const float var = fmaxf(sq * (1.0f / (CELLS * CIN)) - mean * mean, 0.0f);
-                const float rstd = rsqrtf(var + eps);
-#pragma unroll
-                for (int q = 0; q < 4; ++q) {
-                    const f32x2 gq = *reinterpret_cast<const f32x2 *>(&s_gam[ck * 8 + 2 * q]);
-                    const f32x2 bq = *reinterpret_cast<const f32x2 *>(&s_bet[ck * 8 + 2 * q]);
-                    sc[q] = gq * f32x2{rstd, rstd};
-                    sh[q] = bq - sc[q] * f32x2{mean, mean};
-                }
-            }
-#pragma unroll
-            for (int i = 0; i < PER; ++i) {
-                const int s = lane_t + 64 * i;
-                if (s < VPS) {
-                    V8 out = raw[i];
-                    if (NORM) {
-#pragma unroll
-                        for (int q = 0; q < 4; ++q) {
-                            const f32x2 f = __builtin_elementwise_fma(unpack2(raw[i].w[q]), sc[q], sh[q]);
-                            out.w[q] = pack2(f.x, f.y);
-                        }
-                    }
-                    *reinterpret_cast<V8 *>(img + img_off[i]) = out;
-                }
-            }
-        }
-        stamp(0);
-        lds_barrier();
-        stamp(1);
-        if (tile + gridDim.x < ntiles) {
-            stage_tile(tile + gridDim.x, par ^ 1, lane_t);
-            if (EMBED) load_planes(tile + gridDim.x, lane_t);
-        }
-
-        uint32_t col[3][KPT];
-        {
-            const uint32_t pc = static_cast<uint32_t>(2 * th * PCELLS + l15 + 9 - PCOLS - 1);
-#pragma unroll
-            for (int d = 0; d < 3; ++d) {
-                const uint32_t p = pc + d;
-                const uint32_t o = (p * CELLB + ((l4 ^ (p & 7)) << 4)) & 0xffffu;
-#pragma unroll
-                for (int ks = 0; ks < KPT; ++ks) col[d][ks] = o ^ (ks << 6);
-            }
-        }
-        auto fetch = [&](int it, int tap, bf16x8 (&xf)[KPT]) {
-            const int dy = tap / 3, d = tap % 3;
-            const int disp = (dy * PCOLS + (it / 3) * PCELLS + (it % 3) * 16) * CELLB;
-#pragma unroll
-            for (int ks = 0; ks < KPT; ++ks)
-                xf[ks] = *reinterpret_cast<const bf16x8 *>(&smem[col[d][ks] + disp]);
-        };
-        struct Epi { V8 *slot; V8 rr, o; f32x2 t, v; };
-        auto epi_begin = [&](int it, Epi &e) {
-            const int smp = 2 * th + it / 3, t = (it % 3) * 16 + l15;
-            const int cell = (t >> 3) * COLS + (t & 7);
-            const uint32_t m = (t & 7) == 7 ? 0xffffffffu : 0u;
-            const uint32_t off_real = static_cast<uint32_t>(outt - smem) + smp * OSB + cell * 128 + (((mh * 4 + l4) ^ (cell & 7)) << 4);
-            const uint32_t off_dump = static_cast<uint32_t>(dump - smem) + (wave * 8 + (l15 >> 3) + 2 * l4) * 16;
-            e.slot = reinterpret_cast<V8 *>(&smem[(off_real & ~m) | (off_dump & m)]);
-            if (RESID) e.rr = *e.slot;
-        };
-        auto epi_step = [&](int step, const f32x4 (&acc)[2], Epi &e) {
-            const int q = step / 9;
-            const f32x2 x = {acc[q >> 1][2 * (q & 1)], acc[q >> 1][2 * (q & 1) + 1]};
-            switch (step % 9) {
-            case 0: e.t = x * f32x2{-1.44269504f, -1.44269504f}; break;
-            case 1: e.t.x = __builtin_amdgcn_exp2f(e.t.x); break;
-            case 2: e.t.y = __builtin_amdgcn_exp2f(e.t.y); break;
-            case 3: e.t += f32x2{1.0f, 1.0f}; break;
-            case 4: e.t.x = __builtin_amdgcn_rcpf(e.t.x); break;
-            case 5: e.t.y = __builtin_amdgcn_rcpf(e.t.y); break;
-            case 6: e.v = x * e.t; break;
-            case 7: if (RESID) e.v += unpack2(e.rr.w[q]); break;
-            default: e.o.w[q] = pack2(e.v.x, e.v.y); break;
-            }
-        };
-        auto epi_end = [&](Epi &e) { *e.slot = e.o; };
-
-        auto block = [&](int it, f32x4 (&acc)[2], bool with_epi, const f32x4 (&pacc)[2]) {
-#pragma unroll
-            for (int mt = 0; mt < 2; ++mt) acc[mt] = f32x4{bia[mt][0], bia[mt][1], bia[mt][2], bia[mt][3]};
-            Epi e;
-            if (with_epi) epi_begin(it - 1, e);
-            bf16x8 xa[KPT], xb[KPT];
-            fetch(it, 0, xa);
-            __builtin_amdgcn_sched_barrier(0);
-#pragma unroll
-            for (int tap = 0; tap < 9; ++tap) {
-                bf16x8 (&cur)[KPT] = (tap & 1) ? xb : xa;
-                bf16x8 (&nxt)[KPT] = (tap & 1) ? xa : xb;
-                if (tap + 1 < 9) fetch(it, tap + 1, nxt);
-                __builtin_amdgcn_sched_barrier(0);
-#pragma unroll
-                for (int ks = 0; ks < KPT; ++ks)
-#pragma unroll
-                    for (int mt = 0; mt < 2; ++mt) {
-                        const int s = tap * KPT + ks;
-                        acc[mt] = __builtin_amdgcn_mfma_f32_16x16x32_bf16(aw[mt][s], cur[ks], acc[mt], 0, 0, 0);
-                        if (with_epi) {
-                            __builtin_amdgcn_sched_barrier(0);
-                            constexpr int PER_SLOT = 36 / (18 * KPT);
-                            const int slot = (tap * KPT + ks) * 2 + mt;
-#pragma unroll
-                            for (int j = 0; j < PER_SLOT; ++j) epi_step(slot * PER_SLOT + j, pacc, e);
-                            __builtin_amdgcn_sched_barrier(0);
-                        }
-                    }
-            }
-            if (with_epi) epi_end(e);
-        };
-        if (!(dbg & 1)) {
-            if ((dbg >> 5) & 3) {
-                if (((dbg >> 5) & 3) == 1) __builtin_amdgcn_s_setprio(1);
-                else if (((dbg >> 5) & 3) == 2) __builtin_amdgcn_s_setprio(2);
-                else __builtin_amdgcn_s_setprio(3);
-            }
-            f32x4 acc_a[2], acc_b[2];
-            block(0, acc_a, false, acc_b);
-            block(1, acc_b, true, acc_a);
-            block(2, acc_a, true, acc_b);
-            block(3, acc_b, true, acc_a);
-            block(4, acc_a, true, acc_b);
-            block(5, acc_b, true, acc_a);
-            {
-                Epi e;
-                epi_begin(5, e);
-#pragma unroll
-                for (int step = 0; step < 36; ++step) epi_step(step, acc_b, e);
-                epi_end(e);
-            }
-            if ((dbg >> 5) & 3) __builtin_amdgcn_s_setprio(0);
-        }
-        stamp(2);
-        asm volatile("s_waitcnt vmcnt(0)" ::: "memory");
-        stamp(3);
-        lds_barrier();
-        stamp(4);
-
-        if (b0 + wave < B && !(dbg & 2)) {
-            uint16_t *ys = y + (b0 + wave) * (CELLS * COUT);
-#pragma unroll
-            for (int i = 0; i < OPER; ++i) {
-                const int s = lane_t + 64 * i;
-                if (s < OVPS) {
-                    const int cell = s >> 3;
-                    const V8 v = *reinterpret_cast<const V8 *>(outt + wave * OSB + s * 16);
-                    *reinterpret_cast<V8 *>(ys + cell * COUT + (((s & 7) ^ (cell & 7)) << 3)) = v;
-                }
-            }
-        }
-        stamp(5);
-    }
-    if (prof && lane == 0 && blockIdx.x < 512)
-        for (int k = 0; k < 6; ++k) g_prof[(blockIdx.x * 4 + wave) * 8 + k] = tp[k];
+__global__ void __launch_bounds__(256, 2) k_stem_conv_block(StemIn st, const uint16_t *w, const uint16_t *bias,
+                                                            const uint16_t *gamma, const uint16_t *beta, uint16_t *y,
+                                                            int64_t B, float eps, int dbg, const int64_t *batch_dev)
+{
+    constexpr int CIN = 64;
+    constexpr bool NORM = true, RESID = true, EMBED = false, STEM = true;
+    const uint16_t *x = nullptr;
+    const EmbedIn em{};
+#include "nn_conv_body.h"
 }
 
 int g_dbg = 0;
@@ -406,6 +100,33 @@
     return 0;
 }
 
+int launch_stem(const StemIn &st, const void *w, const void *bias, const void *gamma, const void *beta, void *y, int64_t B,
+                float eps, const int64_t *batch_dev, hipStream_t s)
+{
+    constexpr size_t smem = static_cast<size_t>(TS) * PCELLS * CELLB + static_cast<size_t>(TS) * CELLS * 64 * 2 +
+                            2 * 64 * sizeof(float) + 512 + PMAPB + FRAGB;
+    static_assert(2 * smem <= 160 * 1024, "two workgroups per CU");
+    auto kern = k_stem_conv_block;
+    static DeviceSetup setup;
+    if (setup.cus({reinterpret_cast<const void *>(kern)}, static_cast<int>(smem), [&] {
+            if (getenv("AZ_NN_VERBOSE") != nullptr) {
+                int per_cu = 0;
+                (void)hipOccupancyMaxActiveBlocksPerMultiprocessor(&per_cu, reinterpret_cast<const void *>(kern), 256, smem);
+                fprintf(stderr, "[az_nn] stem + conv block: %zu B LDS, %d workgroups per CU\n", smem, per_cu);
+            }
+        }) == 0)
+        return 2;
+    static const int prio = [] { const char *e = getenv("AZ_NN_CONV_PRIO"); const int v = e ? atoi(e) : 1; return v < 0 || v > 3 ? 1 : v; }();
+    const int64_t ntiles = (B + TS - 1) / TS;
+    static const int64_t max_grid = getenv("AZ_NN_CONV_GRID") ? atoll(getenv("AZ_NN_CONV_GRID")) : 512;
+    const unsigned grid = static_cast<unsigned>(ntiles < max_grid ? ntiles : max_grid);
+    hipLaunchKernelGGL(kern, dim3(grid), dim3(256), smem, s, st, static_cast<const uint16_t *>(w),
+                       static_cast<const uint16_t *>(bias), static_cast<const uint16_t *>(gamma),
+                       static_cast<const uint16_t *>(beta), static_cast<uint16_t *>(y), B, eps,
+                       g_dbg | (((g_dbg >> 5) & 3) ? 0 : (prio << 5)), batch_dev);
+    return 0;
+}
+
 }
 
 extern "C" {
@@ -431,6 +152,19 @@
     return 1;
 }
 
+int az_nn_stem_conv_block_positions(const az_nn_positions *positions, const void *w_frag, const float *pmap,
+                                    const void *weight_ohwi, const void *bias, const void *gamma, const void *beta, void *y,
+                                    int64_t batch, float eps, const int32_t *gather, const int64_t *batch_dev, void *stream)
+{
+    if (batch <= 0 || positions == nullptr || !positions->bb_p1 || !positions->bb_p2 || !positions->turn || !positions->sym ||
+        w_frag == nullptr || pmap == nullptr || weight_ohwi == nullptr || bias == nullptr || gamma == nullptr || beta == nullptr ||
+        y == nullptr)
+        return 1;
+    const StemIn st{positions->bb_p1, positions->bb_p2, positions->turn, positions->sym, gather,
+                    static_cast<const uint16_t *>(w_frag), pmap};
+    return launch_stem(st, weight_ohwi, bias, gamma, beta, y, batch, eps, batch_dev, static_cast<hipStream_t>(stream));
+}
+
 int az_nn_stem_embed(const float *features, const void *emb_own, const void *emb_opp, const void *pos,
                      const void *weight_ohwi, const void *bias, void *y, int64_t batch, const int32_t *gather,
                      const int64_t *batch_dev, void *stream)
diff --git a/alphazero-al_amd/csrc/nn_conv_body.h b/alphazero-al_amd/csrc/nn_conv_body.h
--- /dev/null
+++ b/alphazero-al_amd/csrc/nn_conv_body.h
@@ -0,0 +1,433 @@
+    static_assert(!EMBED || (CIN == 32 && !NORM && !RESID), "the embedding is fused into the stem only");
+    static_assert(!STEM || (CIN == 64 && NORM && RESID && !EMBED), "the folded stem is fused into the first residual block only");
+    constexpr int NRAW = STEM ? 1 : 2;
+    const int64_t rows_total = B;
+    if (batch_dev != nullptr && *batch_dev < B) B = *batch_dev;
+    constexpr int K = 9 * CIN;
+    constexpr int KSTEPS = K / 32;
+    constexpr int KPT = CIN / 32;
+    constexpr int VPC = CIN / 8;
+    constexpr int VPS = CELLS * VPC;
+    constexpr int PER = (VPS + 63) / 64;
+    constexpr int SB = VPS * 16;
+    constexpr int OVPS = CELLS * COUT / 8;
+    constexpr int OPER = (OVPS + 63) / 64;
+    constexpr int OSB = OVPS * 16;
+
+    extern __shared__ __align__(16) uint8_t smem[];
+    uint8_t *img = smem;
+    uint8_t *rawb = smem + TS * PCELLS * CELLB;
+    uint8_t *outs = rawb + NRAW * TS * SB;
+    float *s_gam = reinterpret_cast<float *>(outs + (RESID ? 0 : TS * OSB)), *s_bet = s_gam + CIN;
+    uint8_t *dump = reinterpret_cast<uint8_t *>(s_gam + 2 * CIN);
+    uint8_t *s_pm = dump + 512, *s_fr = s_pm + PMAPB;
+
+    const int tid = threadIdx.x;
+    const int lane = tid & 63;
+    const int wave = __builtin_amdgcn_readfirstlane(tid >> 6);
+    const int mh = wave & 1, th = wave >> 1;
+    const int l15 = lane & 15, l4 = lane >> 4;
+
+    bf16x8 aw[2][KSTEPS];
+    float bia[2][4];
+#pragma unroll
+    for (int mt = 0; mt < 2; ++mt) {
+        const int o = mh * 32 + (l15 >> 2) * 8 + mt * 4 + (l15 & 3);
+#pragma unroll
+        for (int s = 0; s < KSTEPS; ++s)
+            aw[mt][s] = *reinterpret_cast<const bf16x8 *>(w + static_cast<size_t>(o) * K + s * 32 + l4 * 8);
+#pragma unroll
+        for (int r = 0; r < 4; ++r)
+            bia[mt][r] = __uint_as_float(static_cast<uint32_t>(bias[mh * 32 + l4 * 8 + mt * 4 + r]) << 16);
+    }
+    if (NORM && tid < CIN) {
+        s_gam[tid] = __uint_as_float(static_cast<uint32_t>(gamma[tid]) << 16);
+        s_bet[tid] = __uint_as_float(static_cast<uint32_t>(beta[tid]) << 16);
+    }
+    {
+        V8 z; z.w[0] = z.w[1] = z.w[2] = z.w[3] = 0;
+        constexpr int NV = (TS * PCELLS * CELLB + NRAW * TS * SB) / 16;
+        for (int i = tid; i < NV; i += 256) reinterpret_cast<V8 *>(smem)[i] = z;
+    }
+    if (STEM) {
+        for (int i = tid; i < PMAPB / 16; i += 256) reinterpret_cast<V8 *>(s_pm)[i] = reinterpret_cast<const V8 *>(st.pmap)[i];
+        for (int i = tid; i < FRAGB / 16; i += 256) reinterpret_cast<V8 *>(s_fr)[i] = reinterpret_cast<const V8 *>(st.wfrag)[i];
+    }
+    __syncthreads();
+
+    auto swz_in = [](int cell) { return VPC == 8 ? (cell & 7) : 0; };
+    const uint32_t raw_lds = lds_addr(rawb);
+    if (EMBED) {
+        for (int i = tid; i < CELLS * CIN / 8; i += 256)
+            reinterpret_cast<V8 *>(rawb)[i] = reinterpret_cast<const V8 *>(em.pos)[i];
+        __syncthreads();
+    }
+    auto stage_tile = [&](int64_t tile, int buf, int lane) {
+        const int64_t b = tile * TS + wave;
+        if (EMBED || STEM || b >= B) return;
+        const uint16_t *xs = x + b * (CELLS * CIN);
+#pragma unroll
+        for (int i = 0; i < PER; ++i) {
+            const int s = lane + 64 * i;
+            if (s < VPS) {
+                const int cell = s / VPC;
+                glds16(xs + (cell * VPC + ((s % VPC) ^ swz_in(cell))) * 8, raw_lds + (buf * TS + wave) * SB + i * 1024);
+            }
+        }
+    };
+
+    const int64_t ntiles = (B + TS - 1) / TS;
+    float pl_own[PER], pl_opp[PER];
+    auto load_planes = [&](int64_t tile, int lane) {
+        const int64_t b = tile * TS + wave;
+        const bool live = b < B;
+        int64_t row = !live ? 0 : (em.gather != nullptr ? em.gather[b] : b);
+        if (row < 0 || row >= rows_total) row = 0;
+        if (em.features != nullptr) {
+            const float *fs = em.features + row * (3 * CELLS);
+#pragma unroll
+            for (int i = 0; i < PER; ++i) {
+                const int s = lane + 64 * i;
+                const bool ok = live && s < VPS;
+                pl_own[i] = ok ? fs[s / VPC] : 0.0f;
+                pl_opp[i] = ok ? fs[CELLS + s / VPC] : 0.0f;
+            }
+        } else {
+            const bool p1 = em.turn[row] > 0, mir = em.sym[row] != 0;
+            const uint64_t own = p1 ? em.bb_p1[row] : em.bb_p2[row], opp = p1 ? em.bb_p2[row] : em.bb_p1[row];
+#pragma unroll
+            for (int i = 0; i < PER; ++i) {
+                const int s = lane + 64 * i;
+                const bool ok = live && s < VPS;
+                const int cell = ok ? s / VPC : 0;
+                const int r = cell / COLS, c = cell - r * COLS;
+                const int bit = (mir ? COLS - 1 - c : c) * 7 + (5 - r);
+                pl_own[i] = (ok && ((own >> bit) & 1ull)) ? 1.0f : 0.0f;
+                pl_opp[i] = (ok && ((opp >> bit) & 1ull)) ? 1.0f : 0.0f;
+            }
+        }
+    };
+    auto request_row = [&](int64_t tile) {
+        const int64_t b = tile * TS + wave;
+        int32_t r = 0;
+        if (tile < ntiles && b < B && st.gather != nullptr) r = st.gather[b];
+        return r;
+    };
+    auto request_pos = [&](int64_t tile, int32_t rowv, int lane) {
+        const int64_t b = tile * TS + wave;
+        uint32_t v = 0;
+        if (tile < ntiles && b < B) {
+            int64_t row = st.gather != nullptr ? static_cast<int64_t>(__builtin_amdgcn_readfirstlane(rowv)) : b;
+            if (row < 0 || row >= rows_total) row = 0;
+            const uint32_t *p1 = reinterpret_cast<const uint32_t *>(st.bb_p1 + row), *p2 = reinterpret_cast<const uint32_t *>(st.bb_p2 + row);
+            const uint32_t *src = lane < 2 ? p1 + lane
+                                : lane < 4 ? p2 + (lane - 2)
+                                : lane == 4 ? reinterpret_cast<const uint32_t *>(st.turn + row) : reinterpret_cast<const uint32_t *>(st.sym + row);
+            if (lane < 6) v = *src;
+        }
+        return v;
+    };
+    int32_t rowv = 0;
+    uint32_t posv = 0;
+    if (STEM) {
+        rowv = request_row(blockIdx.x);
+        posv = request_pos(blockIdx.x, rowv, lane);
+        rowv = request_row(static_cast<int64_t>(blockIdx.x) + gridDim.x);
+    }
+    if (EMBED && static_cast<int64_t>(blockIdx.x) < ntiles) load_planes(blockIdx.x, lane);
+    if (static_cast<int64_t>(blockIdx.x) < ntiles) stage_tile(blockIdx.x, 0, lane);
+    asm volatile("s_waitcnt vmcnt(0)" ::: "memory");
+    lds_barrier();
+    int par = 0;
+    const bool prof = dbg & 16;
+    unsigned long long tp[7] = {0, 0, 0, 0, 0, 0, 0}, tl = prof ? __builtin_amdgcn_s_memtime() : 0;
+    auto stamp = [&](int k) {
+        if (prof) {
+            const unsigned long long now = __builtin_amdgcn_s_memtime();
+            tp[k] += now - tl;
+            tl = now;
+        }
+    };
+    uint32_t img_off[PER];
+#pragma unroll
+    for (int i = 0; i < PER; ++i) {
+        const int sl = lane + 64 * i;
+        const int cell = sl / VPC;
+        const int r = cell / COLS, c = cell - r * COLS;
+        const int p = (r + 1) * PCOLS + (c + 1);
+        const int ck = (lane % VPC) ^ swz_in(lane / VPC);
+        img_off[i] = static_cast<uint32_t>((wave * PCELLS + p) * CELLB + ((ck ^ (p & 7)) << 4));
+    }
+    for (int64_t tile = blockIdx.x; tile < ntiles; tile += gridDim.x, par ^= 1) {
+        const int64_t b0 = tile * TS;
+        uint8_t *rawt = rawb + (STEM ? 0 : par) * TS * SB;
+        uint8_t *outt = RESID ? rawt : outs;
+        int lane_t = lane;
+        asm volatile("" : "+v"(lane_t));
+
+        if (STEM) {
+            const uint32_t w0 = __builtin_amdgcn_readlane(posv, 0), w1 = __builtin_amdgcn_readlane(posv, 1);
+            const uint32_t w2 = __builtin_amdgcn_readlane(posv, 2), w3 = __builtin_amdgcn_readlane(posv, 3);
+            const bool p1 = static_cast<int32_t>(__builtin_amdgcn_readlane(posv, 4)) > 0, mir = __builtin_amdgcn_readlane(posv, 5) != 0;
+            if (b0 + wave < B) {
+                const uint64_t bb1 = (static_cast<uint64_t>(w1) << 32) | w0, bb2 = (static_cast<uint64_t>(w3) << 32) | w2;
+                const uint64_t own = p1 ? bb1 : bb2, opp = p1 ? bb2 : bb1;
+                const int g = lane_t >> 4, tl = lane_t & 15;
+                const int my_r = lane_t / COLS, my_c = lane_t - my_r * COLS;
+                const int bit = (mir ? COLS - 1 - my_c : my_c) * 7 + (5 - my_r);
+                const bool own_here = lane_t < CELLS && ((own >> bit) & 1ull);
+                const bool opp_here = lane_t < CELLS && ((opp >> bit) & 1ull);
+                const uint64_t om8 = __ballot(own_here) << 8, pm8 = __ballot(opp_here) << 8;
+                int sh[4];
+#pragma unroll
+                for (int j = 0; j < 4; ++j) {
+                    const int tp4 = g * 4 + j;
+                    sh[j] = tp4 < 9 ? (tp4 / 3) * 7 + tp4 % 3 : 31;
+                }
+                bf16x8 bq[3];
+                int tok[3];
+#pragma unroll
+                for (int tt = 0; tt < 3; ++tt) {
+                    const int token = tt * 16 + tl;
+                    tok[tt] = token;
+                    const int c = token % COLS;
+                    uint32_t m = 0x1C387u;
+                    if (c == 0) m &= ~0x4081u;
+                    if (c == COLS - 1) m &= ~0x10204u;
+                    const uint32_t cmask = token < CELLS ? m : 0u;
+                    const uint32_t wo = static_cast<uint32_t>(om8 >> token) & cmask;
+                    const uint32_t wp = static_cast<uint32_t>(pm8 >> token) & cmask;
+                    uint32_t d[4];
+#pragma unroll
+                    for (int j = 0; j < 4; ++j)
+                        d[j] = (((wo >> sh[j]) & 1u) | (((wp >> sh[j]) & 1u) << 16)) * 0x3F80u;
+                    bq[tt] = __builtin_bit_cast(bf16x8, uint4{d[0], d[1], d[2], d[3]});
+                }
+                const float *s_p = reinterpret_cast<const float *>(s_pm);
+#pragma unroll
+                for (int m = 0; m < 2; ++m) {
+                    const bf16x8 h0 = *reinterpret_cast<const bf16x8 *>(s_fr + ((0 * 4 + 2 * m) * 64 + lane_t) * 16);
+                    const bf16x8 h1 = *reinterpret_cast<const bf16x8 *>(s_fr + ((0 * 4 + 2 * m + 1) * 64 + lane_t) * 16);
+                    const bf16x8 l0 = *reinterpret_cast<const bf16x8 *>(s_fr + ((1 * 4 + 2 * m) * 64 + lane_t) * 16);
+                    const bf16x8 l1 = *reinterpret_cast<const bf16x8 *>(s_fr + ((1 * 4 + 2 * m + 1) * 64 + lane_t) * 16);
+                    const int ch = m * 32 + g * 8;
+#pragma unroll
+                    for (int tt = 0; tt < 3; ++tt) {
+                        f32x4 a0 = *reinterpret_cast<const f32x4 *>(&s_p[tok[tt] * PROW + ch]);
+                        f32x4 a1 = *reinterpret_cast<const f32x4 *>(&s_p[tok[tt] * PROW + ch + 4]);
+                        a0 = MFMA32(h0, bq[tt], a0);
+                        a1 = MFMA32(h1, bq[tt], a1);
+                        a0 = MFMA32(l0, bq[tt], a0);
+                        a1 = MFMA32(l1, bq[tt], a1);
+                        const f32x2 s0 = silu2(f32x2{a0[0], a0[1]}), s1 = silu2(f32x2{a0[2], a0[3]});
+                        const f32x2 s2 = silu2(f32x2{a1[0], a1[1]}), s3 = silu2(f32x2{a1[2], a1[3]});
+                        V8 o;
+                        o.w[0] = pack2(s0.x, s0.y); o.w[1] = pack2(s1.x, s1.y); o.w[2] = pack2(s2.x, s2.y); o.w[3] = pack2(s3.x, s3.y);
+                        if (tt < 2 || tok[tt] < CELLS)
+                            *reinterpret_cast<V8 *>(rawt + wave * SB + tok[tt] * 128 + (((4 * m + g) ^ (tok[tt] & 7)) << 4)) = o;
+                    }
+                }
+            }
+            stamp(6);
+        }
+        {
+            const int ck = (lane_t % VPC) ^ swz_in(lane_t / VPC);
+            V8 raw[PER];
+            if (EMBED) {
+                const V8 eo = *reinterpret_cast<const V8 *>(em.emb_own + ck * 8), ep = *reinterpret_cast<const V8 *>(em.emb_opp + ck * 8);
+#pragma unroll
+                for (int i = 0; i < PER; ++i) {
+                    const int s = lane_t + 64 * i;
+                    if (s < VPS) {
+                        const V8 ps = *reinterpret_cast<const V8 *>(rawb + s * 16);
+                        const f32x2 own = {pl_own[i], pl_own[i]}, opp = {pl_opp[i], pl_opp[i]};
+#pragma unroll
+                        for (int q = 0; q < 4; ++q) {
+                            const f32x2 v = unpack2(ps.w[q]) + own * unpack2(eo.w[q]) + opp * unpack2(ep.w[q]);
+                            raw[i].w[q] = pack2(v.x, v.y);
+                        }
+                    } else {
+                        raw[i].w[0] = raw[i].w[1] = raw[i].w[2] = raw[i].w[3] = 0;
+                    }
+                }
+            } else {
+#pragma unroll
+                for (int i = 0; i < PER; ++i) {
+                    const int s = lane_t + 64 * i;
+                    if (s < VPS) raw[i] = *reinterpret_cast<const V8 *>(rawt + wave * SB + s * 16);
+                    else raw[i].w[0] = raw[i].w[1] = raw[i].w[2] = raw[i].w[3] = 0;
+                }
+            }
+            f32x2 sc[4], sh[4];
+            if (NORM) {
+                f32x2 sum2 = {0.0f, 0.0f}, sq2 = {0.0f, 0.0f};
+#pragma unroll
+                for (int i = 0; i < PER; ++i) {
+#pragma unroll
+                    for (int q = 0; q < 4; ++q) {
+                        const f32x2 f = unpack2(raw[i].w[q]);
+                        sum2 += f;
+                        sq2 = __builtin_elementwise_fma(f, f, sq2);
+                    }
+                }
+                const float sum = wave_sum(sum2.x + sum2.y), sq = wave_sum(sq2.x + sq2.y);
+                const float mean = sum * (1.0f / (CELLS * CIN));
+                const float var = fmaxf(sq * (1.0f / (CELLS * CIN)) - mean * mean, 0.0f);
+                const float rstd = rsqrtf(var + eps);
+#pragma unroll
+                for (int q = 0; q < 4; ++q) {
+                    const f32x2 gq = *reinterpret_cast<const f32x2 *>(&s_gam[ck * 8 + 2 * q]);
+                    const f32x2 bq = *reinterpret_cast<const f32x2 *>(&s_bet[ck * 8 + 2 * q]);
+                    sc[q] = gq * f32x2{rstd, rstd};
+                    sh[q] = bq - sc[q] * f32x2{mean, mean};
+                }
+            }
+#pragma unroll
+            for (int i = 0; i < PER; ++i) {
+                const int s = lane_t + 64 * i;
+                if (s < VPS) {
+                    V8 out = raw[i];
+                    if (NORM) {
+#pragma unroll
+                        for (int q = 0; q < 4; ++q) {
+                            const f32x2 f = __builtin_elementwise_fma(unpack2(raw[i].w[q]), sc[q], sh[q]);
+                            out.w[q] = pack2(f.x, f.y);
+                        }
+                    }
+                    *reinterpret_cast<V8 *>(img + img_off[i]) = out;
+                }
+            }
+        }
+        stamp(0);
+        lds_barrier();
+        stamp(1);
+        if (tile + gridDim.x < ntiles) {
+            stage_tile(tile + gridDim.x, par ^ 1, lane_t);
+            if (EMBED) load_planes(tile + gridDim.x, lane_t);
+        }
+        if (STEM) {
+            posv = request_pos(tile + gridDim.x, rowv, lane_t);
+            rowv = request_row(tile + 2 * static_cast<int64_t>(gridDim.x));
+        }
+
+        uint32_t col[3][KPT];
+        {
+            const uint32_t pc = static_cast<uint32_t>(2 * th * PCELLS + l15 + 9 - PCOLS - 1);
+#pragma unroll
+            for (int d = 0; d < 3; ++d) {
+                const uint32_t p = pc + d;
+                const uint32_t o = (p * CELLB + ((l4 ^ (p & 7)) << 4)) & 0xffffu;
+#pragma unroll
+                for (int ks = 0; ks < KPT; ++ks) col[d][ks] = o ^ (ks << 6);
+            }
+        }
+        auto fetch = [&](int it, int tap, bf16x8 (&xf)[KPT]) {
+            const int dy = tap / 3, d = tap % 3;
+            const int disp = (dy * PCOLS + (it / 3) * PCELLS + (it % 3) * 16) * CELLB;
+#pragma unroll
+            for (int ks = 0; ks < KPT; ++ks)
+                xf[ks] = *reinterpret_cast<const bf16x8 *>(&smem[col[d][ks] + disp]);
+        };
+        struct Epi { V8 *slot; V8 rr, o; f32x2 t, v; };
+        auto epi_begin = [&](int it, Epi &e) {
+            const int smp = 2 * th + it / 3, t = (it % 3) * 16 + l15;
+            const int cell = (t >> 3) * COLS + (t & 7);
+            const uint32_t m = (t & 7) == 7 ? 0xffffffffu : 0u;
+            const uint32_t off_real = static_cast<uint32_t>(outt - smem) + smp * OSB + cell * 128 + (((mh * 4 + l4) ^ (cell & 7)) << 4);
+            const uint32_t off_dump = static_cast<uint32_t>(dump - smem) + (wave * 8 + (l15 >> 3) + 2 * l4) * 16;
+            e.slot = reinterpret_cast<V8 *>(&smem[(off_real & ~m) | (off_dump & m)]);
+            if (RESID) e.rr = *e.slot;
+        };
+        auto epi_step = [&](int step, const f32x4 (&acc)[2], Epi &e) {
+            const int q = step / 9;
+            const f32x2 x = {acc[q >> 1][2 * (q & 1)], acc[q >> 1][2 * (q & 1) + 1]};
+            switch (step % 9) {
+            case 0: e.t = x * f32x2{-1.44269504f, -1.44269504f}; break;
+            case 1: e.t.x = __builtin_amdgcn_exp2f(e.t.x); break;
+            case 2: e.t.y = __builtin_amdgcn_exp2f(e.t.y); break;
+            case 3: e.t += f32x2{1.0f, 1.0f}; break;
+            case 4: e.t.x = __builtin_amdgcn_rcpf(e.t.x); break;
+            case 5: e.t.y = __builtin_amdgcn_rcpf(e.t.y); break;
+            case 6: e.v = x * e.t; break;
+            case 7: if (RESID) e.v += unpack2(e.rr.w[q]); break;
+            default: e.o.w[q] = pack2(e.v.x, e.v.y); break;
+            }
+        };
+        auto epi_end = [&](Epi &e) { *e.slot = e.o; };
+
+        auto block = [&](int it, f32x4 (&acc)[2], bool with_epi, const f32x4 (&pacc)[2]) {
+#pragma unroll
+            for (int mt = 0; mt < 2; ++mt) acc[mt] = f32x4{bia[mt][0], bia[mt][1], bia[mt][2], bia[mt][3]};
+            Epi e;
+            if (with_epi) epi_begin(it - 1, e);
+            bf16x8 xa[KPT], xb[KPT];
+            fetch(it, 0, xa);
+            __builtin_amdgcn_sched_barrier(0);
+#pragma unroll
+            for (int tap = 0; tap < 9; ++tap) {
+                bf16x8 (&cur)[KPT] = (tap & 1) ? xb : xa;
+                bf16x8 (&nxt)[KPT] = (tap & 1) ? xa : xb;
+                if (tap + 1 < 9) fetch(it, tap + 1, nxt);
+                __builtin_amdgcn_sched_barrier(0);
+#pragma unroll
+                for (int ks = 0; ks < KPT; ++ks)
+#pragma unroll
+                    for (int mt = 0; mt < 2; ++mt) {
+                        const int s = tap * KPT + ks;
+                        acc[mt] = __builtin_amdgcn_mfma_f32_16x16x32_bf16(aw[mt][s], cur[ks], acc[mt], 0, 0, 0);
+                        if (with_epi) {
+                            __builtin_amdgcn_sched_barrier(0);
+                            constexpr int PER_SLOT = 36 / (18 * KPT);
+                            const int slot = (tap * KPT + ks) * 2 + mt;
+#pragma unroll
+                            for (int j = 0; j < PER_SLOT; ++j) epi_step(slot * PER_SLOT + j, pacc, e);
+                            __builtin_amdgcn_sched_barrier(0);
+                        }
+                    }
+            }
+            if (with_epi) epi_end(e);
+        };
+        if (!(dbg & 1)) {
+            if ((dbg >> 5) & 3) {
+                if (((dbg >> 5) & 3) == 1) __builtin_amdgcn_s_setprio(1);
+                else if (((dbg >> 5) & 3) == 2) __builtin_amdgcn_s_setprio(2);
+                else __builtin_amdgcn_s_setprio(3);
+            }
+            f32x4 acc_a[2], acc_b[2];
+            block(0, acc_a, false, acc_b);
+            block(1, acc_b, true, acc_a);
+            block(2, acc_a, true, acc_b);
+            block(3, acc_b, true, acc_a);
+            block(4, acc_a, true, acc_b);
+            block(5, acc_b, true, acc_a);
+            {
+                Epi e;
+                epi_begin(5, e);
+#pragma unroll
+                for (int step = 0; step < 36; ++step) epi_step(step, acc_b, e);
+                epi_end(e);
+            }
+            if ((dbg >> 5) & 3) __builtin_amdgcn_s_setprio(0);
+        }
+        stamp(2);
+        asm volatile("s_waitcnt vmcnt(0)" ::: "memory");
+        stamp(3);
+        lds_barrier();
+        stamp(4);
+
+        if (b0 + wave < B && !(dbg & 2)) {
+            uint16_t *ys = y + (b0 + wave) * (CELLS * COUT);
+#pragma unroll
+            for (int i = 0; i < OPER; ++i) {
+                const int s = lane_t + 64 * i;
+                if (s < OVPS) {
+                    const int cell = s >> 3;
+                    const V8 v = *reinterpret_cast<const V8 *>(outt + wave * OSB + s * 16);
+                    *reinterpret_cast<V8 *>(ys + cell * COUT + (((s & 7) ^ (cell & 7)) << 3)) = v;
+                }
+            }
+        }
+        stamp(5);
+    }
+    if (prof && lane == 0 && blockIdx.x < 512)
+        for (int k = 0; k < (STEM ? 7 : 6); ++k) g_prof[(blockIdx.x * 4 + wave) * 8 + k] = tp[k];
diff --git a/alphazero-al_amd/csrc/nn_model.hip b/alphazero-al_amd/csrc/nn_model.hip
--- a/alphazero-al_amd/csrc/nn_model.hip
+++ b/alphazero-al_amd/csrc/nn_model.hip
@@ -13,6 +13,7 @@
 struct az_nn_model {
     int kind = AZ_NN_KIND_CONNECT4_CNN;
     bool attn_heads_fused = true;
+    bool stem_fused = true;
     az_nn_model_weights w{};
     az_nn_othello_weights ow{};
 };
@@ -163,6 +164,8 @@
     m->w = *w;
     const char *fused = getenv("AZ_ATTN_HEADS_FUSED");
     m->attn_heads_fused = fused == nullptr || strcmp(fused, "0") != 0;
+    const char *stem = getenv("AZ_STEM_FUSED");
+    m->stem_fused = stem == nullptr || strcmp(stem, "0") != 0;
     *out = m;
     return 0;
 }
@@ -303,18 +306,25 @@
     }
     auto begin = [&](int kd) { if (timed && slot[kd] >= 0) (void)hipEventRecord(g_prof.start[kd][slot[kd]], hs); };
     auto end = [&](int kd) { if (timed && slot[kd] >= 0) (void)hipEventRecord(g_prof.stop[kd][slot[kd]], hs); };
-    begin(AZ_NN_PROFILE_STEM);
     int rc;
-    if (w.stem_frag != nullptr && w.stem_pmap != nullptr)
-        rc = positions != nullptr
-            ? az_nn_stem_folded_positions(positions, w.stem_frag, w.stem_pmap, a, batch, rows, n_rows, stream)
-            : az_nn_stem_folded(features, w.stem_frag, w.stem_pmap, a, batch, rows, n_rows, stream);
-    else
-        rc = positions != nullptr
-            ? az_nn_stem_embed_positions(positions, w.emb_own, w.emb_opp, w.pos, w.stem_w, w.stem_b, a, batch, rows, n_rows, stream)
-            : az_nn_stem_embed(features, w.emb_own, w.emb_opp, w.pos, w.stem_w, w.stem_b, a, batch, rows, n_rows, stream);
-    end(AZ_NN_PROFILE_STEM);
-    for (int i = 0; rc == 0 && i < w.n_blocks; ++i) {
+    int first = 0;
+    if (m->stem_fused && !timed && positions != nullptr && w.stem_frag != nullptr && w.stem_pmap != nullptr && w.n_blocks >= 1) {
+        rc = az_nn_stem_conv_block_positions(positions, w.stem_frag, w.stem_pmap, w.block_w[0], w.block_b[0], w.block_gamma[0],
+                                             w.block_beta[0], a, batch, w.eps, rows, n_rows, stream);
+        first = 1;
+    } else {
+        begin(AZ_NN_PROFILE_STEM);
+        if (w.stem_frag != nullptr && w.stem_pmap != nullptr)
+            rc = positions != nullptr
+                ? az_nn_stem_folded_positions(positions, w.stem_frag, w.stem_pmap, a, batch, rows, n_rows, stream)
+                : az_nn_stem_folded(features, w.stem_frag, w.stem_pmap, a, batch, rows, n_rows, stream);
+        else
+            rc = positions != nullptr
+                ? az_nn_stem_embed_positions(positions, w.emb_own, w.emb_opp, w.pos, w.stem_w, w.stem_b, a, batch, rows, n_rows, stream)
+                : az_nn_stem_embed(features, w.emb_own, w.emb_opp, w.pos, w.stem_w, w.stem_b, a, batch, rows, n_rows, stream);
+        end(AZ_NN_PROFILE_STEM);
+    }
+    for (int i = first; rc == 0 && i < w.n_blocks; ++i) {
         if (i == 0) begin(AZ_NN_PROFILE_CONV);
         rc = az_nn_conv_block(a, 64, w.block_w[i], w.block_b[i], w.block_gamma[i], w.block_beta[i], 1, b, batch,
                               w.eps, n_rows, stream);
diff --git a/alphazero-al_amd/src/fast_net.py b/alphazero-al_amd/src/fast_net.py
--- a/alphazero-al_amd/src/fast_net.py
+++ b/alphazero-al_amd/src/fast_net.py
@@ -31,6 +31,7 @@
                                            vp, vp]
             L.az_nn_stem_embed.argtypes = [vp, vp, vp, vp, vp, vp, vp, i64, vp, vp, vp]
             L.az_nn_stem_folded.argtypes = [vp, vp, vp, vp, i64, vp, vp, vp]
+            L.az_nn_stem_conv_block_positions.argtypes = [C.POINTER(Positions), vp, vp, vp, vp, vp, vp, vp, i64, f32, vp, vp, vp]
             L.az_nn_model_create.argtypes = [C.POINTER(ModelWeights), C.POINTER(vp)]
             L.az_nn_model_destroy.argtypes = [vp]
             L.az_nn_model_destroy.restype = None
@@ -79,6 +80,10 @@
     pmap = torch.zeros((48, 68), dtype=torch.float32, device=w.device)
     pmap[:CELLS, :out_c] = pm.reshape(out_c, CELLS).t()
     return frag, pmap.contiguous()
+
+
+class Positions(C.Structure):
+    _fields_ = [(n, C.c_void_p) for n in ("bb_p1", "bb_p2", "turn", "sym")]
 
 
 class HeadsWeights(C.Structure):
diff --git a/include/az_nn.h b/include/az_nn.h
--- a/include/az_nn.h
+++ b/include/az_nn.h
@@ -34,6 +34,9 @@
                       const int32_t *gather, const int64_t *batch_dev, void *stream);
 int az_nn_stem_folded_positions(const az_nn_positions *positions, const void *w_frag, const float *pmap, void *y,
                                 int64_t batch, const int32_t *gather, const int64_t *batch_dev, void *stream);
+int az_nn_stem_conv_block_positions(const az_nn_positions *positions, const void *w_frag, const float *pmap,
+                                    const void *weight_ohwi, const void *bias, const void *gamma, const void *beta, void *y,
+                                    int64_t batch, float eps, const int32_t *gather, const int64_t *batch_dev, void *stream);
 int az_nn_attn_block(const void *x, const void *prenorm_w, const void *qkvg_w, const void *q_norm_w,
                      const void *k_norm_w, const void *o_w, void *y, int64_t batch, float eps, const int64_t *batch_dev,
                      void *stream);
```
